# ErickRosete/tacorl

Hardware: AMD Instinct MI355X
Metric: offline grad-steps/sec (batch=256, 84x84 RGB) (higher is better)
Workload: dtype bf16; 1 GPU; tacorl actor-critic training_step, frozen LMP (BASELINE configs[1]); per_gpu_batch=256, global_batch=256, window=16, image=84x84x3, frames=fp32 CHW (reference batch schema), latent_plan=16, n_action_samples=4, phase=Q (epoch>=bc_epochs), action_decoder_loss=every step (reference behaviour), parallelism=dp1, hip_graph=True, losses_finite=True

## Files before the change

include/tacorl_hip.h:

```cpp
#ifndef TACORL_HIP_H
#define TACORL_HIP_H
#include <stddef.h>
#ifdef __cplusplus
extern "C" {
#endif

typedef void* tacorl_stream_t;

#define TACORL_MAXP 16
enum { TACORL_F32 = 0, TACORL_BF16 = 1 };
enum { TACORL_ACT_NONE = 0, TACORL_ACT_RELU = 1, TACORL_ACT_SILU = 2, TACORL_ACT_TANH = 3 };

int tacorl_hip_version(void);
int tacorl_hip_init(int device);
const char* tacorl_hip_last_error(void);
int tacorl_time_mark(unsigned long long* marks, int slot, tacorl_stream_t stream);
int tacorl_time_spin(unsigned long long* marks, int slot, long ticks, tacorl_stream_t stream);

int tacorl_linear_fwd(int nprob, const float* const* x, int ldx, const float* const* w,
                      const float* const* b, float* const* y, float* const* z, const int* M,
                      int K, int N, int act, int compute_dtype, tacorl_stream_t stream);
size_t tacorl_linear_add_fwd_ws_bytes(int nprob, const int* M, int K, int N);
int tacorl_linear_add_fwd(int nprob, const float* const* x, int ldx, const float* const* w,
                          const float* const* b, const float* const* addend, int ld_add, float* const* y,
// ... 105 lines not shown
int tacorl_encoder_bwd_fused_head(int nprob, const float* const* params, const float* const* act,
                                  const float* const* d_out, const int* n_img, int H, int W,
                                  int prepacked, void* ws, size_t ws_bytes, tacorl_stream_t stream);
int tacorl_encoder_bwd_fused_fc_wgrad(int nprob, const float* const* act, const float* const* d_out,
                                      float* const* grads, const int* n_img, int H, int W,
                                      int accumulate, void* ws, size_t ws_bytes, tacorl_stream_t stream);
int tacorl_encoder_bwd_fused_conv(int nprob, const void* const* img, const float* const* params,
                                  const float* const* act, float* const* grads, const int* n_img, int H,
                                  int W, int accumulate, int prepacked, void* ws, size_t ws_bytes,
                                  tacorl_stream_t stream);
int tacorl_encoder_bwd_fused_conv_parts(int nprob, const void* const* img, const float* const* params,
                                        const float* const* act, float* const* grads, const int* n_img, int H,
                                        int W, int accumulate, int prepacked, int parts, void* ws,
                                        size_t ws_bytes, tacorl_stream_t stream);

long tacorl_mlp_param_layout(int n_layers, const int* dims, long* w_off, long* b_off);
long tacorl_mlp_act_layout(int M, int n_layers, const int* dims, const int* acts, long* z_off,
                           long* y_off);
int tacorl_mlp_fwd(int nprob, const float* const* x, int ldx, const float* const* params,
                   float* const* act, const int* M, int n_layers, const int* dims,
                   const int* acts, int compute_dtype, tacorl_stream_t stream);
int tacorl_mlp_fwd_fused_supported(int nprob, int n_layers, const int* dims, int ldx);
int tacorl_mlp_lean_supported(int nprob, int n_layers, const int* dims, int ldx, int ldo, int ldd);
int tacorl_mlp_fwd_fused(int nprob, const float* const* x, int ldx, const float* const* params,
                         const void* const* params_bf16, float* const* act, const int* M,
                         int n_layers, const int* dims, const int* acts, int lean, tacorl_stream_t stream);
int tacorl_mlp_fwd_fused_gather_supported(int nprob, const int* M, int n_layers, const int* dims, const int* acts,
                                          int ldx, int lean);
int tacorl_mlp_fwd_fused_gather(int nprob, const int* nseg, const float* const* seg_ptr, const int* seg_ld,
                                const int* seg_c0, const int* seg_mod, float* const* x_out, int ldx,
                                const float* const* params, const void* const* params_bf16, float* const* act,
                                const int* M, int n_layers, const int* dims, const int* acts, int lean,
                                tacorl_stream_t stream);
int tacorl_to_bf16_batch(int n, const float* const* src, void* const* dst, const long* count,
                         tacorl_stream_t stream);
size_t tacorl_mlp_bwd_ws_bytes(int nprob, const int* M, int n_layers, const int* dims);
int tacorl_mlp_bwd(int nprob, const float* const* x, int ldx, const float* const* params,
                   const float* const* act, const float* const* d_out, int ldo, float* const* grads,
                   float* const* d_x, int ldd, const int* M, int n_layers, const int* dims,
                   const int* acts, int compute_dtype, int accumulate, void* ws, size_t ws_bytes,
                   tacorl_stream_t stream);
int tacorl_mlp_bwd_fused_supported(int nprob, int n_layers, const int* dims, int ldo, int ldd);
size_t tacorl_mlp_bwd_fused_ws_bytes(int nprob, const int* M, int n_layers, const int* dims);
int tacorl_mlp_bwd_fused_dgrad(int nprob, const float* const* params, const float* const* act,
                               const float* const* d_out, int ldo, float* const* d_x, int ldd,
                               const int* M, int n_layers, const int* dims, const int* acts,
                               int prepacked, void* ws, size_t ws_bytes, tacorl_stream_t stream);
int tacorl_mlp_bwd_fused_pack(int nprob, const float* const* params, const int* M, int n_layers,
                              const int* dims, void* ws, size_t ws_bytes, tacorl_stream_t stream);
int tacorl_prep_batch_begin(void);
int tacorl_reduce_batch_begin(void);
int tacorl_reduce_batch_end(tacorl_stream_t stream);
int tacorl_prep_batch_end(tacorl_stream_t stream);
int tacorl_mlp_bwd_fused_wgrad(int nprob, const float* const* x, int ldx, const float* const* act,
                               const float* const* d_out, int ldo, float* const* grads, const int* M,
                               int n_layers, const int* dims, const int* acts, int accumulate, int lean,
                               void* ws, size_t ws_bytes, tacorl_stream_t stream);

int tacorl_pack_images(const float* src, long img_pitch, int src_nchw, void* dst, int dst_dtype,
                       int n, int C, int H, int W, tacorl_stream_t stream);
int tacorl_pack_images_batch(int njobs, const float* const* src, const long* img_pitch, void* const* dst,
                             const int* n_img, int dst_dtype, int H, int W, tacorl_stream_t stream);
int tacorl_pack_images_window_batch(int njobs, const float* const* src, const long* img_pitch, void* const* dst,
                                    const int* n_img, void* const* dst_first, void* const* dst_last,
                                    const int* window, int dst_dtype, int H, int W, tacorl_stream_t stream);
int tacorl_pack_images_u8_batch(int njobs, const void* const* src, const long* img_pitch_bytes, void* const* dst,
                                const int* n_img, int dst_dtype, int H, int W, tacorl_stream_t stream);
int tacorl_pack_images_u8_gather_batch(int njobs, const void* const* src, const long* img_pitch_bytes,
                                       const long* const* index, const int* index_stride, void* const* dst,
                                       const int* n_img, int dst_dtype, int H, int W, tacorl_stream_t stream);
int tacorl_gather_frames_u8(const void* frames, long frame_bytes, const long* index, void* dst, long n,
                            tacorl_stream_t stream);
int tacorl_pack_images_u8_aug_batch(int njobs, const void* const* src, const long* img_pitch_bytes,
                                    void* const* dst, const int* const* shift, const float* const* jitter,
                                    const int* n_img, int dst_dtype, int H, int W, int pad,
                                    tacorl_stream_t stream);
int tacorl_pack_images_u8_resize_aug_gather_batch(int njobs, const void* const* src, const long* img_pitch_bytes,
                                                  const long* const* index, const int* index_stride, void* const* dst,
                                                  const int* const* shift, const float* const* jitter, const int* n_img,
                                                  int dst_dtype, int src_H, int src_W, int H, int W, int pad,
                                                  tacorl_stream_t stream);
int tacorl_pack_images_u8_aug_gather_batch(int njobs, const void* const* src, const long* img_pitch_bytes,
                                           const long* const* index, const int* index_stride, void* const* dst,
                                           const int* const* shift, const float* const* jitter, const int* n_img,
                                           int dst_dtype, int H, int W, int pad, tacorl_stream_t stream);
int tacorl_stage_transition(const void* disp, int disp_dtype, float* reward, float* done, int B,
                            const float* acts_src, float* acts_dst, long n_acts, tacorl_stream_t stream);
int tacorl_sample_transitions(const long* possible_steps, long n_possible, const long* ep_start, const long* ep_end,
                              int n_episodes, const long* nn_ptr, long n_nn, const long* nn_val, const float* actions,
                              const long* idx, const long* strategy, const long* disp, const double* u_choice,
                              long current_horizon, long n_frames, int B, int A, long* ids, float* action,
                              float* reward, float* done, int* status, tacorl_stream_t stream);
int tacorl_sample_relay(const long* episode_lookup, long n_items, const long* ep_start, const long* ep_end, int n_episodes,
                        const float* actions, long n_frames, const long* idx, const double* u_low, const double* u_high,
                        long max_low_level_window, long max_high_level_window, int B, int A, long* ids, float* action,
                        int* status, tacorl_stream_t stream);
int tacorl_sample_d4rl_windows(const long* episode_lookup, long n_items, const long* ep_start, const long* ep_end,
                               int n_episodes, const float* observations, const float* actions, long n_frames,
                               const long* idx, const long* window, const long* disp, int B, int Tmax, int S, int A,
                               int G, int min_window, float threshold, float* obs, float* act, float* goal,
                               float* reached, float* done, long* window_size, long* ids, int* status,
                               tacorl_stream_t stream);
int tacorl_sample_play_windows(const long* episode_lookup, long n_items, const long* ep_start, const long* ep_end,
                               int n_episodes, const long* nn_ptr, long n_nn, const long* nn_val, const float* actions,
                               long n_frames, long last_end, const long* idx, const long* window, const long* strategy,
                               const long* disp, const long* noise_step, const double* u_choice,
                               const double* u_random_state, int B, int Tmax, int A, int min_window, long* ids, float* act,
                               long* disp_out, long* window_size, int* status, tacorl_stream_t stream);
int tacorl_copy_cols(const float* src, int ld_src, float* dst, int ld_dst, int rows, int cols,
                     int src_row_mod, int accumulate, tacorl_stream_t stream);
int tacorl_copy_cols_batch(int n, const float* const* src, const int* ld_src, float* const* dst,
                           const int* ld_dst, const int* rows, const int* cols,
                           const int* src_row_mod, const int* accumulate, tacorl_stream_t stream);
int tacorl_vec_rows_max_blocks(void);
int tacorl_vec_rows(const float* obs, const float* goal, const float* acts_main, const float* act_pi,
                    const float* act_next, float* const* out, void* const* out_bf16, int B, int T, int S, int G, int A,
                    int n, int lds, int ldq, tacorl_stream_t stream);
int tacorl_reduce_rows_mod(const float* in, int ld_in, float* out, int ld_out, int B, int cols,
                           int reps, tacorl_stream_t stream);
int tacorl_reduce_rows_mod_batch(int n, const float* const* in, int ld_in, float* const* out, int ld_out, int B,
                                 int cols, int reps, tacorl_stream_t stream);
int tacorl_uniform_actions(const float* u01, float* dst, int ld_dst, int rows, int A,
                           int discrete_gripper, tacorl_stream_t stream);

int tacorl_tanh_normal_sample(const float* head, int ld_head, const float* eps, const float* gumbel_u,
                              int hard_rsample, float* act_out, int ld_act, float* logp, int* grip_idx,
                              int n, int M, int Ac, tacorl_stream_t stream);
int tacorl_tanh_normal_sample_batch(int njobs, const float* const* head, int ld_head,
                                    const float* const* eps, const float* const* gumbel_u,
                                    const int* hard_rsample, float* const* act_out, int ld_act,
                                    float* const* logp, int* const* grip_idx, const int* n, int M, int Ac,
                                    const float* u01, float* u_dst, int u_rows, int A, int u_discrete,
                                    tacorl_stream_t stream);

int tacorl_add_rows_bcast(const float* x, int ldx, const float* add, float* out, int R, int T, int D,
                          int Dp, tacorl_stream_t stream);
int tacorl_attention_fwd(const float* qkv, float* out, int B, int T, int D, int H, tacorl_stream_t stream);
int tacorl_attention_dropout_fwd(const float* qkv, float* out, const unsigned char* keep, float keep_scale, int B,
                                 int T, int D, int H, tacorl_stream_t stream);
int tacorl_attention_dropout_bwd(const float* qkv, const float* d_out, float* d_qkv, const unsigned char* keep,
                                 float keep_scale, int B, int T, int D, int H, tacorl_stream_t stream);
int tacorl_dropout_mul(float* x, const unsigned char* keep, float keep_scale, long n, tacorl_stream_t stream);
int tacorl_add_layernorm_fwd(const float* x, const float* res, const float* w, const float* b, float* y,
                             float* stats, int R, int D, float eps, tacorl_stream_t stream);
int tacorl_pr_encoder_fused_supported(int D, int T, int H, int FF, int L);
int tacorl_pr_encoder_fused_train_supported(int D, int T, int H, int FF, int L);
int tacorl_pr_encoder_fused(const float* emb, int ld_emb, const float* params, const void* params_bf16,
                            const long* offsets, float* pooled, int B, int D, int T, int H, int FF, int L,
                            tacorl_stream_t stream);
int tacorl_pr_encoder_fused_sample(const float* emb, int ld_emb, const float* params, const void* params_bf16,
                                   const long* offsets, float* pooled, int B, int D, int T, int H, int FF, int L,
                                   const float* Wc, const float* bc, const float* eps, float* head, float* plan,
                                   int A, float min_std, tacorl_stream_t stream);
int tacorl_pr_encoder_fused_train(const float* emb, int ld_emb, const float* params, const void* params_bf16,
                                  const long* offsets, float* pooled, int B, int D, int T, int H, int FF, int L,
                                  float* const* save, tacorl_stream_t stream);
int tacorl_pr_encoder_bwd_fused(const float* params, const long* offsets, const float* d_pool, const float* d_head,
                                const float* Wc, int A2, float* dx, const float* const* saved, float* const* dz,
                                const void* const* wt, float* ln_part, float* const* ln_grads, int B, int D, int T, int H,
                                int FF, int L, tacorl_stream_t stream);
int tacorl_pr_encoder_fused_train_sample(const float* emb, int ld_emb, const float* params, const void* params_bf16,
                                         const long* offsets, float* pooled, int B, int D, int T, int H, int FF, int L,
                                         float* const* save, const float* Wc, const float* bc, const float* eps,
                                         float* head, float* plan, int A, float min_std, tacorl_stream_t stream);
int tacorl_pr_head_compose(const float* w_fc, const float* b_fc, const float* w_head, const float* b_head,
                           float* Wc, float* bc, int D, int FC, int A2, tacorl_stream_t stream);
int tacorl_mean_over_t(const float* x, float* out, int B, int T, int D, tacorl_stream_t stream);
int tacorl_pr_sample(const float* head, const float* eps, float* plan, float* mu_out, float* std_out,
                     int B, int A, float min_std, tacorl_stream_t stream);

int tacorl_build_ad_input(const float* plan, const float* emb, int ld_emb, float* out, int B, int T,
                          int Tm, int P, int E, tacorl_stream_t stream);
int tacorl_ad_input_proj(const float* plan, const float* emb, int ld_emb, const float* w_ih, const float* b_ih,
                         float* out, int B, int T, int Tm, int P, int E, int H, tacorl_stream_t stream);
size_t tacorl_logistic_mixture_ws_bytes(int B, int Tm, int Da);
int tacorl_logistic_mixture_loss(const float* heads, int ldh, const float* actions, float* d_heads,
                                 float* loss_out, int B, int T, int Tm, int Da, int K, int num_classes,
                                 float gripper_alpha, float grad_scale, void* ws, size_t ws_bytes,
                                 tacorl_stream_t stream);
int tacorl_logistic_mixture_finish(const void* ws, size_t ws_bytes, int B, int Tm, int Da, float* loss_out,
                                   tacorl_stream_t stream);
int tacorl_logistic_mixture_sample(const float* heads, int ldh, const float* rand_a, const float* rand_b,
                                   float* out, int R, int Da, int K, tacorl_stream_t stream);

int tacorl_logistic_mixture_nogrip_loss(const float* heads, int ldh, const float* actions, float* d_heads,
                                        float* loss_out, int B, int T, int Tm, int Da, int K, int num_classes,
                                        float grad_scale, void* ws, size_t ws_bytes, tacorl_stream_t stream);
int tacorl_logistic_mixture_nogrip_finish(const void* ws, size_t ws_bytes, int B, int Tm, int Da, float* loss_out,
                                          tacorl_stream_t stream);
int tacorl_logistic_mixture_nogrip_sample(const float* heads, int ldh, const float* rand_a, const float* rand_b,
                                          float* out, int R, int Da, int K, tacorl_stream_t stream);

int tacorl_relu_mask_mul(const float* dy, const float* add, const float* h, float* out, long n,
                         tacorl_stream_t stream);
int tacorl_ad_input_bwd(const float* dx, float* d_plan, float* d_emb, int ld_emb, int B, int T, int Tm,
                        int P, int E, int accumulate, tacorl_stream_t stream);
int tacorl_plmp_demb_finish(float* d_emb, const float* dx, int ld_dx, int D_in, const float* dS, int ld_ds,
                            const float* dgin, float* const* f_dout, int ncam, int B, int T, int Ec,
                            tacorl_stream_t stream);
int tacorl_bcast_over_t(const float* src, float* dst, int B, int T, int D, float scale, int accumulate,
                        tacorl_stream_t stream);
int tacorl_attention_bwd(const float* qkv, const float* d_out, float* d_qkv, int B, int T, int D, int H,
                         tacorl_stream_t stream);
size_t tacorl_add_layernorm_bwd_ws_bytes(int R, int D);
int tacorl_add_layernorm_bwd(const float* dy, const float* x, const float* res, const float* w,
                             const float* stats, float* dv, float* dw, float* db, int R, int D,
                             int accumulate, void* ws, size_t ws_bytes, tacorl_stream_t stream);
int tacorl_gauss_kl_balanced(const float* head_q, const float* head_p, float* d_head_q, float* d_head_p,
                             int B, int A, float kl_alpha, float kl_beta, float min_std, int balanced,
                             float grad_scale, float* out2, tacorl_stream_t stream);
int tacorl_pr_sample_bwd(const float* head, const float* eps, const float* d_plan, float* d_head, int B,
                         int A, float min_std, tacorl_stream_t stream);

enum {
  TACORL_LG_ALPHA_LOSS = 0, TACORL_LG_ALPHA, TACORL_LG_ACTOR_LOSS, TACORL_LG_BELL1, TACORL_LG_BELL2,
  TACORL_LG_CONS1, TACORL_LG_CONS2, TACORL_LG_Q1LOSS, TACORL_LG_Q2LOSS, TACORL_LG_ALPHA_P,
  TACORL_LG_ALPHA_P_LOSS, TACORL_LG_Q1_DATA, TACORL_LG_Q1_RAND, TACORL_LG_Q1_POL, TACORL_LG_Q2_DATA,
  TACORL_LG_Q2_RAND, TACORL_LG_Q2_POL, TACORL_LG_ACTION_LOSS, TACORL_LG_COUNT
};
int tacorl_alpha_loss(const float* logp, int B, const float* log_alpha, float target_entropy,
                      float grad_scale, float* g_log_alpha, float* logs, tacorl_stream_t stream);
int tacorl_alpha_loss_step(const float* logp, int B, float* log_alpha, float target_entropy, float* g_log_alpha,
                           float* logs, float* m, float* v, float lr, int* step_counter, tacorl_stream_t stream);
int tacorl_actor_qmin(const float* q1, const float* q2, const float* logp, int B, const float* log_alpha,
                      float* dq1, float* dq2, float grad_scale, float* logs, tacorl_stream_t stream);
int tacorl_actor_head_bwd(const float* head, int ld_head, const float* eps, const float* logp,
                          const float* g_act1, const float* g_act2, int ld_g, const float* value,
                          int ld_value, const int* grip_idx, const float* log_alpha, float grad_scale,
                          float* d_head, int B, int Ac, int has_grip, float* logs, tacorl_stream_t stream);
int tacorl_tanh_normal_nll(const float* head, int ld_head, const float* target, int ld_target, int M, int Ac,
                           int has_grip, float grad_scale, float* d_head, float* loss_out, tacorl_stream_t stream);

size_t tacorl_cql_ws_bytes(int B);
int tacorl_cql_loss(const float* q1, const float* q2, float* dq1, float* dq2, const float* tq1,
                    const float* tq2, const float* logp_cur, const float* logp_nxt, const float* next_logp,
                    const float* reward, const float* done, const float* log_alpha,
                    const float* log_alpha_prime, int B, int n, int A, float discount, float reward_scale,
                    float temp, float cons_w, float gap, int deterministic_backup, float grad_scale,
                    float* g_log_alpha_prime, float* logs, void* ws, size_t ws_bytes, tacorl_stream_t stream);

size_t tacorl_adam_ws_bytes(long n);
int tacorl_adam_step(float* param, const float* grad, float* m, float* v, long n, float lr,
                     float max_norm, int* step_counter, float* target, float tau, void* ws,
                     size_t ws_bytes, tacorl_stream_t stream);
size_t tacorl_adam_batch_ws_bytes(int nb);
int tacorl_adam_step_batch(int nb, float* const* param, const float* const* grad, float* const* m,
                           float* const* v, const long* n, const float* lr, const float* max_norm,
                           int* const* step_counter, float* const* target, const float* tau, void* ws,
                           size_t ws_bytes, tacorl_stream_t stream);
int tacorl_adam_step_batch_mirror(int nb, float* const* param, const float* const* grad, float* const* m,
                                  float* const* v, const long* n, const float* lr, const float* max_norm,
                                  int* const* step_counter, float* const* target, const float* tau,
                                  void* const* mirror, void* const* target_mirror, void* ws, size_t ws_bytes,
                                  tacorl_stream_t stream);

int tacorl_cem_supported(int N, int A, int E, int hidden, int q_layers, int compute_dtype);
size_t tacorl_cem_ws_bytes(int R, int N, int A, int E, int hidden, int q_layers, int compute_dtype);
int tacorl_cem_refine(int R, int nnet, const float* const* s, const float* const* params,
                      const void* const* params_bf16, const float* mean0, const float* eps, float* out, int N, int A,
                      int E, int hidden, int q_layers, int iters, int n_elite, float min_std, float max_std, float alpha,
                      int discrete_gripper, int compute_dtype, float* t_pop, float* t_q, int* t_elite, float* t_mean,
                      float* t_std, void* ws, size_t ws_bytes, tacorl_stream_t stream);

int tacorl_knn_l2_supported(int D, int k);
int tacorl_knn_l2_tile(void);
int tacorl_knn_l2_query_block(int k);
int tacorl_knn_l2(const float* points, long n_points, int D, long ld, long q0, long n_queries, int k, int* nbr_row,
                  float* nbr_dist, tacorl_stream_t stream);
int tacorl_nn_margin_filter(const int* nbr_row, long n_queries, int k, long q0, const long* step_of_row, long n_points,
                            long margin, long* nn_steps, int* count, tacorl_stream_t stream);

int tacorl_rows_linear2_supported(int R, int K1, int K2, int N);
int tacorl_rows_linear2_group(void);
int tacorl_rows_linear2_fwd(const float* x1, int ldx1, int K1, const float* w1, const float* b1, const float* x2, int ldx2,
                            int K2, const float* w2, const float* b2, const unsigned char* x2_row_is_zero, float* y, int ldy,
                            int R, int N, int act, tacorl_stream_t stream);

#define TACORL_ROWS_MLP_PLAIN 0
#define TACORL_ROWS_MLP_POLICY_ACTION 1
int tacorl_rows_mlp_supported(int R, int n_layers, const int* dims, int mode, int Ac, int discrete_gripper);
int tacorl_rows_mlp_npw(int N, int R);
int tacorl_rows_mlp_fwd(const float* x, int ldx, int n_layers, const int* dims, const float* const* w, const float* const* b,
                        const int* acts, float* ws, float* y, int ldy, int R, int mode, int Ac, int discrete_gripper, int npw,
                        tacorl_stream_t stream);

#define TACORL_NOISE_MAX_SEGS 64
enum { TACORL_NOISE_NORMAL = 0, TACORL_NOISE_UNIFORM = 1, TACORL_NOISE_KEEP = 2 };
typedef struct {
  int offset, kind, draw_id, n_outer, B_local, inner, outer_major;
  float keep_p;
  int group0, reserved;
} tacorl_noise_seg;
typedef struct {
  int n_f32, n_u8, n_groups, reserved;
  tacorl_noise_seg seg[1];
} tacorl_noise_table;
int tacorl_noise_fill(const void* segs, int n_seg, void* base_f32, void* base_u8, unsigned long long seed, unsigned int step,
                      int sample0, tacorl_stream_t stream);

#ifdef __cplusplus
}
#endif
#endif
```

tacorl_amd/_lib.py:

```python
import ctypes as C
import os

HERE = os.path.dirname(os.path.abspath(__file__))
LIB_PATH = os.environ.get("TACORL_HIP_LIB") or os.path.join(HERE, "lib", "libtacorl_hip.so")

F32, BF16 = 0, 1
ACT_NONE, ACT_RELU, ACT_SILU, ACT_TANH = 0, 1, 2, 3
MAXP = 16

LOG_SLOTS = [
    "alpha_loss", "alpha", "actor_loss", "bellman_q1_loss", "bellman_q2_loss", "conservative_q1_loss",
    "conservative_q2_loss", "q1_loss", "q2_loss", "alpha_prime", "alpha_prime_loss", "q1_data", "q1_random",
    "q1_policy", "q2_data", "q2_random", "q2_policy", "action_loss",
]

_p, _i, _l, _f, _sz = C.c_void_p, C.c_int, C.c_long, C.c_float, C.c_size_t
_SIGS = {
    "tacorl_hip_version": (_i, []),
    "tacorl_hip_init": (_i, [_i]),
    "tacorl_hip_last_error": (C.c_char_p, []),
    "tacorl_time_mark": (_i, [_p, _i, _p]),
    "tacorl_time_spin": (_i, [_p, _i, _l, _p]),
    "tacorl_linear_fwd": (_i, [_i, _p, _i, _p, _p, _p, _p, _p, _i, _i, _i, _i, _p]),
    "tacorl_linear_add_fwd_ws_bytes": (_sz, [_i, _p, _i, _i]),
    "tacorl_linear_add_fwd": (_i, [_i, _p, _i, _p, _p, _p, _i, _p, _i, _p, _i, _i, _i, _i, _p, _sz, _p]),
    "tacorl_rnn_linear_supported": (_i, [_i, _i, _i]),
    "tacorl_rnn_linear_fwd": (_i, [_p, _p, _p, _p, _i, _p, _p, _i, _i, _i, _i, _p]),
    "tacorl_rnn_linear_fwd_batch": (_i, [_i, _p, _p, _p, _p, _i, _p, _p, _i, _i, _i, _p, _p]),
    "tacorl_rnn_linear_fwd_batch_twin": (_i, [_i, _p, _p, _p, _p, _p, _p, _i, _p, _p, _p, _p, _i, _i, _i, _i, _p, _p]),
    "tacorl_rnn_linear_fwd_batch_ext": (_i, [_i, _p, _p, _p, _p, _p, _p, _i, _p, _p, _p, _p, _i, _i, _i, _i, _p, _p, _p, _p, _p, _p]),
    "tacorl_rnn_linear_ld_supported": (_i, [_i, _i, _i, _i, _i]),
    "tacorl_rnn_linear_ld": (_i, [_i, _p, _i, _p, _p, _p, _p, _i, _p, _p, _p, _p, _p, _i, _i, _i, _i, _i, _p]),
    "tacorl_rnn_linear_bwd_step": (_i, [_p, _p, _p, _i, _p, _p, _p, _i, _i, _i, _p]),
    "tacorl_rnn_linear_bwd_batch": (_i, [_i, _p, _p, _p, _i, _p, _p, _p, _i, _i, _i, _p]),
    "tacorl_rnn_wgrad_supported": (_i, [_i, _i, _i]),
    "tacorl_rnn_wgrad": (_i, [_p, _i, _p, _i, _i, _i, _i, _p, _p, _i, _p]),
    "tacorl_rnn_wgrad_batch": (_i, [_i, _p, _i, _p, _i, _p, _i, _i, _p, _p, _i, _p]),
    "tacorl_rnn_wgrad_slabs_ws_bytes": (_sz, [_i, _i, _i]),
    "tacorl_rnn_wgrad_slabs": (_i, [_p, _i, _p, _i, _i, _i, _i, _i, _i, _p, _p, _i, _p, _sz, _p]),
    "tacorl_birnn_swap_rows": (_i, [_p, _i, _p, _i, _i, _i, _i, _p]),
    "tacorl_transpose_to_bf16": (_i, [_p, _p, _i, _i, _p]),
    "tacorl_transpose_to_bf16_batch": (_i, [_i, _p, _p, _p, _p, _p]),
    "tacorl_transpose_pad_to_bf16": (_i, [_p, _p, _i, _i, _i, _p]),
    "tacorl_pad_to_bf16": (_i, [_p, _i, _p, _i, _l, _i, _p]),
    "tacorl_pr_encoder_fused_supported": (_i, [_i, _i, _i, _i, _i]),
    "tacorl_pr_encoder_fused_train_supported": (_i, [_i, _i, _i, _i, _i]),
    "tacorl_pr_encoder_fused": (_i, [_p, _i, _p, _p, _p, _p, _i, _i, _i, _i, _i, _i, _p]),
    "tacorl_pr_encoder_fused_train": (_i, [_p, _i, _p, _p, _p, _p, _i, _i, _i, _i, _i, _i, _p, _p]),
    "tacorl_pr_encoder_bwd_fused": (_i, [_p, _p, _p, _p, _p, _i, _p, _p, _p, _p, _p, _p, _i, _i, _i, _i, _i, _i, _p]),
    "tacorl_pr_encoder_fused_train_sample": (_i, [_p, _i, _p, _p, _p, _p, _i, _i, _i, _i, _i, _i, _p, _p, _p, _p, _p, _p, _i, _f, _p]),
    "tacorl_pr_encoder_fused_sample": (_i, [_p, _i, _p, _p, _p, _p, _i, _i, _i, _i, _i, _i, _p, _p, _p, _p, _p, _i, _f, _p]),
    "tacorl_pr_head_compose": (_i, [_p, _p, _p, _p, _p, _p, _i, _i, _i, _p]),
    "tacorl_to_bf16_batch": (_i, [_i, _p, _p, _p, _p]),
    "tacorl_mlp_bwd_fused_supported": (_i, [_i, _i, _p, _i, _i]),
    "tacorl_mlp_bwd_fused_ws_bytes": (_sz, [_i, _p, _i, _p]),
    "tacorl_mlp_bwd_fused_dgrad": (_i, [_i, _p, _p, _p, _i, _p, _i, _p, _i, _p, _p, _i, _p, _sz, _p]),
    "tacorl_mlp_bwd_fused_pack": (_i, [_i, _p, _p, _i, _p, _p, _sz, _p]),
    "tacorl_prep_batch_begin": (_i, []),
    "tacorl_reduce_batch_begin": (_i, []),
    "tacorl_reduce_batch_end": (_i, [_p]),
    "tacorl_prep_batch_end": (_i, [_p]),
    "tacorl_mlp_bwd_fused_wgrad": (_i, [_i, _p, _i, _p, _p, _i, _p, _p, _i, _p, _p, _i, _i, _p, _sz, _p]),
    "tacorl_mlp_fwd_fused_supported": (_i, [_i, _i, _p, _i]),
    "tacorl_mlp_lean_supported": (_i, [_i, _i, _p, _i, _i, _i]),
    "tacorl_mlp_fwd_fused": (_i, [_i, _p, _i, _p, _p, _p, _p, _i, _p, _p, _i, _p]),
    "tacorl_mlp_fwd_fused_gather_supported": (_i, [_i, _p, _i, _p, _p, _i, _i]),
    "tacorl_mlp_fwd_fused_gather": (_i, [_i, _p, _p, _p, _p, _p, _p, _i, _p, _p, _p, _p, _i, _p, _p, _i, _p]),
    "tacorl_add_rows_bcast": (_i, [_p, _i, _p, _p, _i, _i, _i, _i, _p]),
    "tacorl_attention_fwd": (_i, [_p, _p, _i, _i, _i, _i, _p]),
    "tacorl_attention_dropout_fwd": (_i, [_p, _p, _p, _f, _i, _i, _i, _i, _p]),
    "tacorl_attention_dropout_bwd": (_i, [_p, _p, _p, _p, _f, _i, _i, _i, _i, _p]),
    "tacorl_dropout_mul": (_i, [_p, _p, _f, _l, _p]),
    "tacorl_add_layernorm_fwd": (_i, [_p, _p, _p, _p, _p, _p, _i, _i, _f, _p]),
    "tacorl_mean_over_t": (_i, [_p, _p, _i, _i, _i, _p]),
    "tacorl_pr_sample": (_i, [_p, _p, _p, _p, _p, _i, _i, _f, _p]),
    "tacorl_build_ad_input": (_i, [_p, _p, _i, _p, _i, _i, _i, _i, _i, _p]),
    "tacorl_build_ad_input_bf16": (_i, [_p, _p, _i, _p, _i, _i, _i, _i, _i, _p]),
    "tacorl_ad_input_proj": (_i, [_p, _p, _i, _p, _p, _p, _i, _i, _i, _i, _i, _i, _p]),
    "tacorl_logistic_mixture_ws_bytes": (_sz, [_i, _i, _i]),
    "tacorl_logistic_mixture_loss": (_i, [_p, _i, _p, _p, _p, _i, _i, _i, _i, _i, _i, _f, _f, _p, _sz, _p]),
    "tacorl_logistic_mixture_finish": (_i, [_p, _sz, _i, _i, _i, _p, _p]),
    "tacorl_logistic_mixture_sample": (_i, [_p, _i, _p, _p, _p, _i, _i, _i, _p]),
    "tacorl_logistic_mixture_nogrip_loss": (_i, [_p, _i, _p, _p, _p, _i, _i, _i, _i, _i, _i, _f, _p, _sz, _p]),
    "tacorl_logistic_mixture_nogrip_finish": (_i, [_p, _sz, _i, _i, _i, _p, _p]),
    "tacorl_logistic_mixture_nogrip_sample": (_i, [_p, _i, _p, _p, _p, _i, _i, _i, _p]),
    "tacorl_linear_dgrad": (_i, [_i, _p, _i, _p, _p, _i, _p, _i, _i, _p, _i, _p, _i, _i, _i, _p]),
    "tacorl_linear_dgrad_ws_bytes": (_sz, [_i, _p, _i, _i]),
    "tacorl_linear_dgrad_splitk": (_i, [_i, _p, _i, _p, _p, _i, _p, _i, _i, _p, _i, _p, _i, _i, _i, _p, _sz, _p]),
    "tacorl_linear_wgrad_ws_bytes": (_sz, [_i, _p, _i, _i]),
    "tacorl_linear_wgrad": (_i, [_i, _p, _i, _p, _i, _p, _i, _i, _p, _p, _i, _i, _p, _sz, _p]),
    "tacorl_relu_mask_mul": (_i, [_p, _p, _p, _p, _l, _p]),
    "tacorl_ad_input_bwd": (_i, [_p, _p, _p, _i, _i, _i, _i, _i, _i, _i, _p]),
    "tacorl_plmp_demb_finish": (_i, [_p, _p, _i, _i, _p, _i, _p, _p, _i, _i, _i, _i, _p]),
    "tacorl_bcast_over_t": (_i, [_p, _p, _i, _i, _i, _f, _i, _p]),
    "tacorl_attention_bwd": (_i, [_p, _p, _p, _i, _i, _i, _i, _p]),
    "tacorl_add_layernorm_bwd_ws_bytes": (_sz, [_i, _i]),
    "tacorl_add_layernorm_bwd": (_i, [_p, _p, _p, _p, _p, _p, _p, _p, _i, _i, _i, _p, _sz, _p]),
    "tacorl_gauss_kl_balanced": (_i, [_p, _p, _p, _p, _i, _i, _f, _f, _f, _i, _f, _p, _p]),
    "tacorl_pr_sample_bwd": (_i, [_p, _p, _p, _p, _i, _i, _f, _p]),
    "tacorl_conv2d_relu_fwd": (_i, [_i, _p, _p, _p, _p, _p, _i, _i, _i, _i, _i, _i, _i, _i, _i, _p]),
    "tacorl_encoder_param_layout": (_l, [_p]),
    "tacorl_encoder_act_layout": (_l, [_i, _i, _i, _p]),
    "tacorl_encoder_fwd": (_i, [_i, _p, _p, _p, _p, _p, _i, _i, _i, _i, _p]),
    "tacorl_encoder_bwd_ws_bytes": (_sz, [_i, _p, _i, _i]),
    "tacorl_encoder_bwd": (_i, [_i, _p, _p, _p, _p, _p, _p, _i, _i, _i, _i, _i, _p, _sz, _p]),
    "tacorl_encoder_fused_wpk_bytes": (_l, []),
    "tacorl_encoder_fused_supported": (_i, [_i, _i]),
    "tacorl_encoder_fused_act_format": (_i, [_i, _i]),
    "tacorl_encoder_pack_weights": (_i, [_i, _p, _p, _p]),
    "tacorl_encoder_fwd_fused": (_i, [_i, _p, _p, _p, _p, _p, _p, _i, _i, _p]),
    "tacorl_encoder_fwd_fused_wg": (_i, [_i, _p, _p, _p, _p, _p, _p, _i, _i, _i, _p]),
    "tacorl_encoder_src_entry_bytes": (_l, []),
    "tacorl_encoder_src_supported": (_i, [_p, _l, _l, _l, _i, _i]),
    "tacorl_encoder_src_fill": (_i, [_p, _i, _p, _p, _p, _p, _i, _i, _p]),
    "tacorl_encoder_fwd_fused_src": (_i, [_i, _p, _p, _p, _p, _p, _p, _p, _i, _i, _i, _p]),
    "tacorl_encoder_bwd_fused_ws_bytes": (_sz, [_i, _p, _i, _i]),
    "tacorl_encoder_bwd_fused": (_i, [_i, _p, _p, _p, _p, _p, _p, _i, _i, _i, _p, _sz, _p]),
    "tacorl_encoder_bwd_fused_pack": (_i, [_i, _p, _p, _i, _i, _p, _sz, _p]),
    "tacorl_encoder_bwd_fused_head": (_i, [_i, _p, _p, _p, _p, _i, _i, _i, _p, _sz, _p]),
    "tacorl_encoder_bwd_fused_fc_wgrad": (_i, [_i, _p, _p, _p, _p, _i, _i, _i, _p, _sz, _p]),
    "tacorl_encoder_bwd_fused_conv": (_i, [_i, _p, _p, _p, _p, _p, _i, _i, _i, _i, _p, _sz, _p]),
    "tacorl_encoder_bwd_fused_conv_parts": (_i, [_i, _p, _p, _p, _p, _p, _i, _i, _i, _i, _i, _p, _sz, _p]),
    "tacorl_mlp_param_layout": (_l, [_i, _p, _p, _p]),
    "tacorl_mlp_act_layout": (_l, [_i, _i, _p, _p, _p, _p]),
    "tacorl_mlp_fwd": (_i, [_i, _p, _i, _p, _p, _p, _i, _p, _p, _i, _p]),
    "tacorl_mlp_bwd_ws_bytes": (_sz, [_i, _p, _i, _p]),
    "tacorl_mlp_bwd": (_i, [_i, _p, _i, _p, _p, _p, _i, _p, _p, _i, _p, _i, _p, _p, _i, _i, _p, _sz, _p]),
    "tacorl_pack_images": (_i, [_p, _l, _i, _p, _i, _i, _i, _i, _i, _p]),
    "tacorl_pack_images_batch": (_i, [_i, _p, _p, _p, _p, _i, _i, _i, _p]),
    "tacorl_pack_images_window_batch": (_i, [_i, _p, _p, _p, _p, _p, _p, _p, _i, _i, _i, _p]),
    "tacorl_pack_images_u8_batch": (_i, [_i, _p, _p, _p, _p, _i, _i, _i, _p]),
    "tacorl_pack_images_u8_gather_batch": (_i, [_i, _p, _p, _p, _p, _p, _p, _i, _i, _i, _p]),
    "tacorl_pack_images_u8_aug_gather_batch": (_i, [_i, _p, _p, _p, _p, _p, _p, _p, _p, _i, _i, _i, _i, _p]),
    "tacorl_pack_images_u8_resize_aug_gather_batch": (_i, [_i, _p, _p, _p, _p, _p, _p, _p, _p, _i, _i, _i, _i, _i, _i, _p]),
    "tacorl_gather_frames_u8": (_i, [_p, _l, _p, _p, _l, _p]),
    "tacorl_pack_images_u8_aug_batch": (_i, [_i, _p, _p, _p, _p, _p, _p, _i, _i, _i, _i, _p]),
    "tacorl_stage_transition": (_i, [_p, _i, _p, _p, _i, _p, _p, _l, _p]),
    "tacorl_sample_transitions": (_i, [_p, _l, _p, _p, _i, _p, _l, _p, _p, _p, _p, _p, _p, _l, _l, _i, _i, _p, _p, _p, _p, _p, _p]),
    "tacorl_sample_relay": (_i, [_p, _l, _p, _p, _i, _p, _l, _p, _p, _p, _l, _l, _i, _i, _p, _p, _p, _p]),
    "tacorl_sample_d4rl_windows": (_i, [_p, _l, _p, _p, _i, _p, _p, _l, _p, _p, _p, _i, _i, _i, _i, _i, _i, _f, _p, _p, _p, _p, _p, _p,
                                        _p, _p, _p]),
    "tacorl_sample_play_windows": (_i, [_p, _l, _p, _p, _i, _p, _l, _p, _p, _l, _l, _p, _p, _p, _p, _p, _p, _p, _i, _i, _i, _i,
                                        _p, _p, _p, _p, _p, _p]),
    "tacorl_copy_cols": (_i, [_p, _i, _p, _i, _i, _i, _i, _i, _p]),
    "tacorl_copy_cols_batch": (_i, [_i, _p, _p, _p, _p, _p, _p, _p, _p, _p]),
    "tacorl_vec_rows_max_blocks": (_i, []),
    "tacorl_vec_rows": (_i, [_p, _p, _p, _p, _p, _p, _p, _i, _i, _i, _i, _i, _i, _i, _i, _p]),
    "tacorl_reduce_rows_mod": (_i, [_p, _i, _p, _i, _i, _i, _i, _p]),
    "tacorl_reduce_rows_mod_batch": (_i, [_i, _p, _i, _p, _i, _i, _i, _i, _p]),
    "tacorl_uniform_actions": (_i, [_p, _p, _i, _i, _i, _i, _p]),
    "tacorl_tanh_normal_sample": (_i, [_p, _i, _p, _p, _i, _p, _i, _p, _p, _i, _i, _i, _p]),
    "tacorl_tanh_normal_sample_batch": (_i, [_i, _p, _i, _p, _p, _p, _p, _i, _p, _p, _p, _i, _i, _p, _p, _i, _i, _i, _p]),
    "tacorl_alpha_loss": (_i, [_p, _i, _p, _f, _f, _p, _p, _p]),
    "tacorl_alpha_loss_step": (_i, [_p, _i, _p, _f, _p, _p, _p, _p, _f, _p, _p]),
    "tacorl_actor_qmin": (_i, [_p, _p, _p, _i, _p, _p, _p, _f, _p, _p]),
    "tacorl_actor_head_bwd": (_i, [_p, _i, _p, _p, _p, _p, _i, _p, _i, _p, _p, _f, _p, _i, _i, _i, _p, _p]),
    "tacorl_tanh_normal_nll": (_i, [_p, _i, _p, _i, _i, _i, _i, _f, _p, _p, _p]),
    "tacorl_cql_ws_bytes": (_sz, [_i]),
    "tacorl_cql_loss": (_i, [_p] * 13 + [_i, _i, _i, _f, _f, _f, _f, _f, _i, _f, _p, _p, _p, _sz, _p]),
    "tacorl_adam_ws_bytes": (_sz, [_l]),
    "tacorl_adam_step": (_i, [_p, _p, _p, _p, _l, _f, _f, _p, _p, _f, _p, _sz, _p]),
    "tacorl_adam_batch_ws_bytes": (_sz, [_i]),
    "tacorl_adam_step_batch": (_i, [_i, _p, _p, _p, _p, _p, _p, _p, _p, _p, _p, _p, _sz, _p]),
    "tacorl_adam_step_batch_mirror": (_i, [_i, _p, _p, _p, _p, _p, _p, _p, _p, _p, _p, _p, _p, _p, _sz, _p]),
    "tacorl_cem_supported": (_i, [_i, _i, _i, _i, _i, _i]),
    "tacorl_cem_ws_bytes": (_sz, [_i, _i, _i, _i, _i, _i, _i]),
    "tacorl_cem_refine": (_i, [_i, _i, _p, _p, _p, _p, _p, _p, _i, _i, _i, _i, _i, _i, _i, _f, _f, _f, _i, _i, _p, _p, _p, _p, _p,
                               _p, _sz, _p]),
    "tacorl_knn_l2_supported": (_i, [_i, _i]),
    "tacorl_knn_l2_tile": (_i, []),
    "tacorl_knn_l2_query_block": (_i, [_i]),
    "tacorl_knn_l2": (_i, [_p, _l, _i, _l, _l, _l, _i, _p, _p, _p]),
    "tacorl_nn_margin_filter": (_i, [_p, _l, _i, _l, _p, _l, _l, _p, _p, _p]),
    "tacorl_rows_linear2_supported": (_i, [_i, _i, _i, _i]),
    "tacorl_rows_linear2_group": (_i, []),
    "tacorl_rows_linear2_fwd": (_i, [_p, _i, _i, _p, _p, _p, _i, _i, _p, _p, _p, _p, _i, _i, _i, _i, _p]),
    "tacorl_rows_mlp_supported": (_i, [_i, _i, _p, _i, _i, _i]),
    "tacorl_rows_mlp_npw": (_i, [_i, _i]),
    "tacorl_rows_mlp_fwd": (_i, [_p, _i, _i, _p, _p, _p, _p, _p, _p, _i, _i, _i, _i, _i, _i, _p]),
    "tacorl_noise_fill": (_i, [_p, _i, _p, _p, C.c_ulonglong, C.c_uint, _i, _p]),
}

_lib = None


class TacorlHipError(RuntimeError):
    pass


def lib():
    global _lib
    if _lib is None:
        import torch

        if not os.path.exists(LIB_PATH):
            raise TacorlHipError(
                f"{LIB_PATH} not found: the HIP extension is required (no CPU fallback). "
                "Build it with `python -m tacorl_amd.build`.")
        L = C.CDLL(LIB_PATH)
        override = bool(os.environ.get("TACORL_HIP_LIB"))
        missing = []
        for name, (res, args) in _SIGS.items():
            fn = getattr(L, name, None)
            if fn is None:
# ... 53 lines not shown
```

tacorl_amd/csrc/pr_fused.hip:

```cpp
#include <hip/hip_runtime.h>
#include <stdint.h>

#include "../../include/tacorl_hip.h"
#include "common.h"

namespace {

#ifndef PR_W2TOP
#define PR_W2TOP 0
#endif
constexpr int PR_D = 32, PR_T = 16, PR_H = 8, PR_HD = 4, PR_MAXL = 4, PR_CH = 256;
constexpr int XB_P = 40;
constexpr int HB_P = 264;
constexpr int QKV_P = 100;

struct PrLayerOff { long in_w, in_b, out_w, out_b, w1, b1, w2, b2, n1w, n1b, n2w, n2b; };
struct PrSaveL { float *xin, *qkv, *att, *proj, *x1, *ff1, *ff2, *st1, *st2; };
struct PrArgs {
  const float* emb;
  const float* P;
  const __bf16* Pb;
  float* pooled;
  long pos;
  PrLayerOff l[PR_MAXL];
  int ld_emb, B, FF, L;
  const float* Wc;
  const float* bc;
  const float* eps;
  float* head;
  float* plan;
  int A;
  float min_std;
  PrSaveL sv[PR_MAXL];
  int save;
};

__device__ __forceinline__ bf16x8 cvt8(const float* p) {
  const f32x4 a = *reinterpret_cast<const f32x4*>(p), b = *reinterpret_cast<const f32x4*>(p + 4);
  return bf16x8{(__bf16)a[0], (__bf16)a[1], (__bf16)a[2], (__bf16)a[3], (__bf16)b[0], (__bf16)b[1], (__bf16)b[2], (__bf16)b[3]};
}
__device__ __forceinline__ void lds_sync() { asm volatile("s_waitcnt lgkmcnt(0)" ::: "memory"); }

__device__ __forceinline__ void layer_norm32(f32x4 (&v)[2], const float* w, const float* b, int g, float* st = nullptr) {
  float s = 0.f;
#pragma unroll
  for (int nt = 0; nt < 2; nt++)
#pragma unroll
    for (int r = 0; r < 4; r++) s += v[nt][r];
  s += __shfl_xor(s, 16, 64);
  s += __shfl_xor(s, 32, 64);
  const float mean = s / 32.f;
  float q = 0.f;
#pragma unroll
  for (int nt = 0; nt < 2; nt++)
#pragma unroll
    for (int r = 0; r < 4; r++) { const float c = v[nt][r] - mean; q += c * c; }
  q += __shfl_xor(q, 16, 64);
  q += __shfl_xor(q, 32, 64);
  const float rstd = 1.0f / sqrtf(q / 32.f + 1e-5f);
  if (st && g == 0) { st[0] = mean; st[1] = rstd; }
#pragma unroll
  for (int nt = 0; nt < 2; nt++) {
    const f32x4 ww = *reinterpret_cast<const f32x4*>(w + 16 * nt + 4 * g), bb = *reinterpret_cast<const f32x4*>(b + 16 * nt + 4 * g);
#pragma unroll
    for (int r = 0; r < 4; r++) v[nt][r] = (v[nt][r] - mean) * rstd * ww[r] + bb[r];
  }
}

__device__ __forceinline__ void layer_norm32_r(f32x4 (&v)[2], const f32x4 (&ww)[2], const f32x4 (&bb)[2], int g, float* st = nullptr) {
  float s = 0.f;
#pragma unroll
  for (int nt = 0; nt < 2; nt++)
#pragma unroll
    for (int r = 0; r < 4; r++) s += v[nt][r];
  s += __shfl_xor(s, 16, 64);
  s += __shfl_xor(s, 32, 64);
  const float mean = s / 32.f;
  float q = 0.f;
#pragma unroll
  for (int nt = 0; nt < 2; nt++)
#pragma unroll
    for (int r = 0; r < 4; r++) { const float c = v[nt][r] - mean; q += c * c; }
  q += __shfl_xor(q, 16, 64);
  q += __shfl_xor(q, 32, 64);
  const float rstd = 1.0f / sqrtf(q / 32.f + 1e-5f);
  if (st && g == 0) { st[0] = mean; st[1] = rstd; }
#pragma unroll
  for (int nt = 0; nt < 2; nt++)
#pragma unroll
    for (int r = 0; r < 4; r++) v[nt][r] = (v[nt][r] - mean) * rstd * ww[nt][r] + bb[nt][r];
}

#ifdef PR_STAMPS
__device__ unsigned long long pr_stamps[16];
#define PR_STAMP(k)                                          \
  do {                                                       \
    if (blockIdx.x == 0 && threadIdx.x == 0) {               \
      const unsigned long long t_ = clock64();               \
      atomicAdd(&pr_stamps[k], t_ - t_prev);                 \
      t_prev = t_;                                           \
    }                                                        \
  } while (0)
#else
#define PR_STAMP(k)
#endif

template <int RT>
__global__ __launch_bounds__(256) void pr_encoder_fused_kernel(PrArgs a) {
#ifdef PR_STAMPS
  unsigned long long t_prev = clock64();
#endif
  constexpr int T = 16 * RT;
  __shared__ __attribute__((aligned(16))) __bf16 xb_s[4][T * XB_P];
  __shared__ __attribute__((aligned(16))) unsigned char big_s[4][T * HB_P * 2];
  const int lane = threadIdx.x & 63, w = threadIdx.x >> 6, i = lane & 15, g = lane >> 4;
  __shared__ __attribute__((aligned(16))) float ypart[2][4][T * PR_D];
  constexpr int PR_B1C = 2;
  __shared__ __attribute__((aligned(16))) float b1_s[4][PR_B1C * PR_CH];
  const int b = blockIdx.x;
  if (b >= a.B) return;
  __bf16* xb = xb_s[w];
  float* qkv = reinterpret_cast<float*>(big_s[w]);
  __bf16* hb = reinterpret_cast<__bf16*>(big_s[w]);
  static_assert(T * QKV_P * 4 <= T * HB_P * 2, "q|k|v fits in the hidden-chunk buffer");

  const int A_ = a.A, jh = lane < 2 * A_ ? lane : 0;
  f32x4 hw[PR_D / 4];
  float hbias = 0.f, heps = 0.f;
  if (a.Wc) {
#pragma unroll
    for (int d = 0; d < PR_D / 4; d++) hw[d] = *reinterpret_cast<const f32x4*>(a.Wc + jh * PR_D + 4 * d);
    hbias = a.bc[jh];
    heps = a.eps[(long)b * A_ + (lane < A_ ? lane : 0)];
  }
  f32x4 x[RT][2];
#pragma unroll
  for (int rt = 0; rt < RT; rt++)
#pragma unroll
    for (int nt = 0; nt < 2; nt++) {
      const int n = 16 * nt + 4 * g, t = 16 * rt + i;
      x[rt][nt] = *reinterpret_cast<const f32x4*>(a.emb + ((long)b * T + t) * a.ld_emb + n) +
                  *reinterpret_cast<const f32x4*>(a.P + a.pos + t * PR_D + n);
    }
  auto put_xb = [&](const f32x4 (&v)[RT][2]) {
#pragma unroll
    for (int rt = 0; rt < RT; rt++)
#pragma unroll
      for (int nt = 0; nt < 2; nt++)
        *reinterpret_cast<bf16x4*>(xb + (16 * rt + i) * XB_P + 16 * nt + 4 * g) =
            bf16x4{(__bf16)v[rt][nt][0], (__bf16)v[rt][nt][1], (__bf16)v[rt][nt][2], (__bf16)v[rt][nt][3]};
  };
  const int nchunk = a.FF / PR_CH;
  const bool sv0 = a.save && w == 0;
  long rrow[RT];
#pragma unroll
  for (int rt = 0; rt < RT; rt++) rrow[rt] = (long)b * T + 16 * rt + i;
  for (int l = 0; l < a.L; l++) {
    const PrLayerOff& o = a.l[l];
    const PrSaveL& S = a.sv[l];
    bf16x8 inw[6], outw[2];
    f32x4 inb[6], outb[2], n1w[2], n1b[2], n2w[2], n2b[2], b2v[2];
#pragma unroll
    for (int nt = 0; nt < 6; nt++) {
      inw[nt] = *reinterpret_cast<const bf16x8*>(a.Pb + o.in_w + (long)(16 * nt + i) * PR_D + 8 * g);
      inb[nt] = *reinterpret_cast<const f32x4*>(a.P + o.in_b + 16 * nt + 4 * g);
    }
#pragma unroll
    for (int nt = 0; nt < 2; nt++) {
      outw[nt] = *reinterpret_cast<const bf16x8*>(a.Pb + o.out_w + (long)(16 * nt + i) * PR_D + 8 * g);
      outb[nt] = *reinterpret_cast<const f32x4*>(a.P + o.out_b + 16 * nt + 4 * g);
      n1w[nt] = *reinterpret_cast<const f32x4*>(a.P + o.n1w + 16 * nt + 4 * g);
      n1b[nt] = *reinterpret_cast<const f32x4*>(a.P + o.n1b + 16 * nt + 4 * g);
      n2w[nt] = *reinterpret_cast<const f32x4*>(a.P + o.n2w + 16 * nt + 4 * g);
      n2b[nt] = *reinterpret_cast<const f32x4*>(a.P + o.n2b + 16 * nt + 4 * g);
      b2v[nt] = *reinterpret_cast<const f32x4*>(a.P + o.b2 + 16 * nt + 4 * g);
    }
    const __bf16* W1 = a.Pb + o.w1;
    const __bf16* W2 = a.Pb + o.w2;
    bf16x8 w1f[16], w2f[8][2];
    const int c0 = w < nchunk ? w : nchunk - 1;
#pragma unroll
    for (int nt = 0; nt < 16; nt++) w1f[nt] = *reinterpret_cast<const bf16x8*>(W1 + (long)(PR_CH * c0 + 16 * nt + i) * PR_D + 8 * g);
    f32x4 b1pre[PR_B1C];
    const bool b1_staged = nchunk <= 4 * PR_B1C;
    if (b1_staged) {
#pragma unroll
      for (int j = 0; j < PR_B1C; j++) {
        const int c = w + 4 * j;
        b1pre[j] = *reinterpret_cast<const f32x4*>(a.P + o.b1 + PR_CH * (c < nchunk ? c : c0) + 4 * lane);
      }
    }
    if (RT == 1 && PR_W2TOP) {
#pragma unroll
      for (int ks = 0; ks < 8; ks++)
#pragma unroll
        for (int nt = 0; nt < 2; nt++)
          w2f[ks][nt] = *reinterpret_cast<const bf16x8*>(W2 + (long)(16 * nt + i) * a.FF + PR_CH * c0 + 32 * ks + 8 * g);
    }
    if (sv0) {
#pragma unroll
      for (int rt = 0; rt < RT; rt++)
#pragma unroll
        for (int nt = 0; nt < 2; nt++) *reinterpret_cast<f32x4*>(S.xin + rrow[rt] * PR_D + 16 * nt + 4 * g) = x[rt][nt];
    }
    PR_STAMP(0);
    put_xb(x);
    lds_sync();
    {
      bf16x8 xf[RT];
#pragma unroll
      for (int rt = 0; rt < RT; rt++) xf[rt] = *reinterpret_cast<const bf16x8*>(xb + (16 * rt + i) * XB_P + 8 * g);
#pragma unroll
      for (int nt = 0; nt < 6; nt++) {
        const bf16x8 wf = inw[nt];
        const f32x4 bias = inb[nt];
#pragma unroll
        for (int rt = 0; rt < RT; rt++) {
          f32x4 acc = bias;
          acc = __builtin_amdgcn_mfma_f32_16x16x32_bf16(wf, xf[rt], acc, 0, 0, 0);
          *reinterpret_cast<f32x4*>(qkv + (16 * rt + i) * QKV_P + 16 * nt + 4 * g) = acc;
          if (sv0) *reinterpret_cast<f32x4*>(S.qkv + rrow[rt] * 3 * PR_D + 16 * nt + 4 * g) = acc;
        }
      }
    }
    lds_sync();
    PR_STAMP(1);
#pragma unroll
    for (int j = 0; j < 2 * RT; j++) {
      const int p = lane + 64 * j, h = p / T, qi = p % T;
      f32x4 q = *reinterpret_cast<const f32x4*>(qkv + qi * QKV_P + PR_HD * h);
#pragma unroll
      for (int e = 0; e < 4; e++) q[e] *= 0.5f * 1.44269504088896341f;
      float s[T], mx = -INFINITY;
#pragma unroll
      for (int t = 0; t < T; t++) {
        const f32x4 k = *reinterpret_cast<const f32x4*>(qkv + t * QKV_P + PR_D + PR_HD * h);
        s[t] = ((q[0] * k[0] + q[1] * k[1]) + q[2] * k[2]) + q[3] * k[3];
        mx = fmaxf(mx, s[t]);
      }
      float se = 0.f;
#pragma unroll
      for (int t = 0; t < T; t++) { s[t] = __builtin_amdgcn_exp2f(s[t] - mx); se += s[t]; }
      const float rse = __builtin_amdgcn_rcpf(se);
      f32x4 ov = {0.f, 0.f, 0.f, 0.f};
#pragma unroll
      for (int t = 0; t < T; t++) {
        const f32x4 vv = *reinterpret_cast<const f32x4*>(qkv + t * QKV_P + 2 * PR_D + PR_HD * h);
        const float pr = s[t] * rse;
#pragma unroll
        for (int e = 0; e < 4; e++) ov[e] += pr * vv[e];
      }
      *reinterpret_cast<bf16x4*>(xb + qi * XB_P + PR_HD * h) = bf16x4{(__bf16)ov[0], (__bf16)ov[1], (__bf16)ov[2], (__bf16)ov[3]};
      if (sv0) *reinterpret_cast<f32x4*>(S.att + ((long)b * T + qi) * PR_D + PR_HD * h) = ov;
    }
    lds_sync();
    PR_STAMP(2);
    {
      bf16x8 af[RT];
#pragma unroll
      for (int rt = 0; rt < RT; rt++) af[rt] = *reinterpret_cast<const bf16x8*>(xb + (16 * rt + i) * XB_P + 8 * g);
#pragma unroll
      for (int nt = 0; nt < 2; nt++) {
        const bf16x8 wf = outw[nt];
        const f32x4 bias = outb[nt];
#pragma unroll
        for (int rt = 0; rt < RT; rt++) {
          f32x4 acc = bias;
          acc = __builtin_amdgcn_mfma_f32_16x16x32_bf16(wf, af[rt], acc, 0, 0, 0);
          if (sv0) *reinterpret_cast<f32x4*>(S.proj + rrow[rt] * PR_D + 16 * nt + 4 * g) = acc;
          x[rt][nt] += acc;
        }
      }
#pragma unroll
      for (int rt = 0; rt < RT; rt++) {
        layer_norm32_r(x[rt], n1w, n1b, g, sv0 ? S.st1 + 2 * rrow[rt] : nullptr);
        if (sv0) {
#pragma unroll
          for (int nt = 0; nt < 2; nt++) *reinterpret_cast<f32x4*>(S.x1 + rrow[rt] * PR_D + 16 * nt + 4 * g) = x[rt][nt];
        }
      }
    }
    lds_sync();
    put_xb(x);
    lds_sync();
    PR_STAMP(3);
    if (b1_staged) {
#pragma unroll
      for (int j = 0; j < PR_B1C; j++) *reinterpret_cast<f32x4*>(b1_s[w] + PR_CH * j + 4 * lane) = b1pre[j];
      lds_sync();
    }
    bf16x8 xf[RT];
#pragma unroll
    for (int rt = 0; rt < RT; rt++) xf[rt] = *reinterpret_cast<const bf16x8*>(xb + (16 * rt + i) * XB_P + 8 * g);
    f32x4 y[RT][2];
#pragma unroll
    for (int rt = 0; rt < RT; rt++)
#pragma unroll
      for (int nt = 0; nt < 2; nt++)
        y[rt][nt] = w == 0 ? b2v[nt] : f32x4{0.f, 0.f, 0.f, 0.f};
    for (int c = w; c < nchunk; c += 4) {
      if (RT != 1 || !PR_W2TOP || c != w) {
#pragma unroll
        for (int ks = 0; ks < 8; ks++)
#pragma unroll
          for (int nt = 0; nt < 2; nt++)
            w2f[ks][nt] = *reinterpret_cast<const bf16x8*>(W2 + (long)(16 * nt + i) * a.FF + PR_CH * c + 32 * ks + 8 * g);
      }
#pragma unroll
      for (int nt = 0; nt < 16; nt++) {
        const f32x4 bias = b1_staged ? *reinterpret_cast<const f32x4*>(b1_s[w] + PR_CH * ((c - w) >> 2) + 16 * nt + 4 * g)
                                     : *reinterpret_cast<const f32x4*>(a.P + o.b1 + PR_CH * c + 16 * nt + 4 * g);
#pragma unroll
        for (int rt = 0; rt < RT; rt++) {
          f32x4 hacc = bias;
          hacc = __builtin_amdgcn_mfma_f32_16x16x32_bf16(w1f[nt], xf[rt], hacc, 0, 0, 0);
          const f32x4 hr = {fmaxf(hacc[0], 0.f), fmaxf(hacc[1], 0.f), fmaxf(hacc[2], 0.f), fmaxf(hacc[3], 0.f)};
          *reinterpret_cast<bf16x4*>(hb + (16 * rt + i) * HB_P + 16 * nt + 4 * g) = bf16x4{(__bf16)hr[0], (__bf16)hr[1], (__bf16)hr[2], (__bf16)hr[3]};
          if (a.save) *reinterpret_cast<f32x4*>(S.ff1 + rrow[rt] * a.FF + PR_CH * c + 16 * nt + 4 * g) = hr;
        }
      }
      lds_sync();
      if (c + 4 < nchunk) {
#pragma unroll
        for (int nt = 0; nt < 16; nt++)
          w1f[nt] = *reinterpret_cast<const bf16x8*>(W1 + (long)(PR_CH * (c + 4) + 16 * nt + i) * PR_D + 8 * g);
      }
#pragma unroll
      for (int ks = 0; ks < 8; ks++) {
#pragma unroll
        for (int rt = 0; rt < RT; rt++) {
          const bf16x8 hf = *reinterpret_cast<const bf16x8*>(hb + (16 * rt + i) * HB_P + 32 * ks + 8 * g);
#pragma unroll
          for (int nt = 0; nt < 2; nt++) y[rt][nt] = __builtin_amdgcn_mfma_f32_16x16x32_bf16(w2f[ks][nt], hf, y[rt][nt], 0, 0, 0);
        }
      }
      lds_sync();
    }
    PR_STAMP(4);
    {
      float* yp = ypart[l & 1][w];
#pragma unroll
      for (int rt = 0; rt < RT; rt++)
#pragma unroll
        for (int nt = 0; nt < 2; nt++) *reinterpret_cast<f32x4*>(yp + (16 * rt + i) * PR_D + 16 * nt + 4 * g) = y[rt][nt];
      __syncthreads();
#pragma unroll
      for (int rt = 0; rt < RT; rt++)
#pragma unroll
        for (int nt = 0; nt < 2; nt++) {
          f32x4 t = *reinterpret_cast<const f32x4*>(ypart[l & 1][0] + (16 * rt + i) * PR_D + 16 * nt + 4 * g);
#pragma unroll
          for (int ww = 1; ww < 4; ww++) t += *reinterpret_cast<const f32x4*>(ypart[l & 1][ww] + (16 * rt + i) * PR_D + 16 * nt + 4 * g);
          if (sv0) *reinterpret_cast<f32x4*>(S.ff2 + rrow[rt] * PR_D + 16 * nt + 4 * g) = t;
          x[rt][nt] += t;
        }
    }
#pragma unroll
    for (int rt = 0; rt < RT; rt++) layer_norm32_r(x[rt], n2w, n2b, g, sv0 ? S.st2 + 2 * rrow[rt] : nullptr);
    PR_STAMP(5);
  }
  if (w != 0) return;
#pragma unroll
  for (int nt = 0; nt < 2; nt++) {
    f32x4 s = x[0][nt];
#pragma unroll
    for (int rt = 1; rt < RT; rt++) s += x[rt][nt];
#pragma unroll
    for (int off = 1; off < 16; off <<= 1)
#pragma unroll
      for (int r = 0; r < 4; r++) s[r] += __shfl_xor(s[r], off, 64);
    if (i == 0) {
#pragma unroll
      for (int r = 0; r < 4; r++) s[r] *= (1.0f / T);
      *reinterpret_cast<f32x4*>(a.pooled + (long)b * PR_D + 16 * nt + 4 * g) = s;
      if (a.Wc) *reinterpret_cast<f32x4*>(qkv + 16 * nt + 4 * g) = s;
    }
  }
  if (!a.Wc) return;
  lds_sync();
  const int A = A_;
  float h = hbias;
#pragma unroll
  for (int d = 0; d < PR_D; d += 4) {
    const f32x4 wv = hw[d / 4], pv = *reinterpret_cast<const f32x4*>(qkv + d);
    h += wv[0] * pv[0] + wv[1] * pv[1] + wv[2] * pv[2] + wv[3] * pv[3];
  }
  if (lane < 2 * A) a.head[(long)b * 2 * A + lane] = h;
  const float vr = __shfl(h, (lane + A) & 63, 64);
  if (lane < A) {
    const float sd = (vr > 20.f ? vr : log1pf(expf(vr))) + a.min_std;
    a.plan[(long)b * A + lane] = tanhf(h + heps * sd);
  }
}

constexpr int D6 = 64, HD6 = 8, CH6 = 128;
constexpr int XB6_P = 72;
constexpr int HB6_P = 136;
constexpr int QKV6_P = 196;

__device__ __forceinline__ void layer_norm64(f32x4 (&v)[4], const float* w, const float* b, int g) {
  float s = 0.f;
#pragma unroll
  for (int nt = 0; nt < 4; nt++)
#pragma unroll
    for (int r = 0; r < 4; r++) s += v[nt][r];
  s += __shfl_xor(s, 16, 64);
  s += __shfl_xor(s, 32, 64);
  const float mean = s / 64.f;
  float q = 0.f;
#pragma unroll
  for (int nt = 0; nt < 4; nt++)
#pragma unroll
    for (int r = 0; r < 4; r++) { const float c = v[nt][r] - mean; q += c * c; }
  q += __shfl_xor(q, 16, 64);
  q += __shfl_xor(q, 32, 64);
  const float rstd = 1.0f / sqrtf(q / 64.f + 1e-5f);
#pragma unroll
  for (int nt = 0; nt < 4; nt++) {
    const f32x4 ww = *reinterpret_cast<const f32x4*>(w + 16 * nt + 4 * g), bb = *reinterpret_cast<const f32x4*>(b + 16 * nt + 4 * g);
#pragma unroll
    for (int r = 0; r < 4; r++) v[nt][r] = (v[nt][r] - mean) * rstd * ww[r] + bb[r];
  }
}

__device__ __forceinline__ void layer_norm64(f32x4 (&v)[4], const f32x4 (&ww)[4], const f32x4 (&bb)[4]) {
  float s = 0.f;
#pragma unroll
  for (int nt = 0; nt < 4; nt++)
#pragma unroll
    for (int r = 0; r < 4; r++) s += v[nt][r];
  s += __shfl_xor(s, 16, 64);
  s += __shfl_xor(s, 32, 64);
  const float mean = s / 64.f;
  float q = 0.f;
#pragma unroll
  for (int nt = 0; nt < 4; nt++)
#pragma unroll
    for (int r = 0; r < 4; r++) { const float c = v[nt][r] - mean; q += c * c; }
  q += __shfl_xor(q, 16, 64);
  q += __shfl_xor(q, 32, 64);
  const float rstd = 1.0f / sqrtf(q / 64.f + 1e-5f);
#pragma unroll
  for (int nt = 0; nt < 4; nt++)
#pragma unroll
    for (int r = 0; r < 4; r++) v[nt][r] = (v[nt][r] - mean) * rstd * ww[nt][r] + bb[nt][r];
}

template <int RT>
__global__ __launch_bounds__(256) void pr_encoder_fused64_kernel(PrArgs a) {
#ifdef PR_STAMPS
  unsigned long long t_prev = clock64();
#endif
  constexpr int T = 16 * RT;
  constexpr int BIG = (T * QKV6_P * 4 > T * HB6_P * 2) ? T * QKV6_P * 4 : T * HB6_P * 2;
  __shared__ __attribute__((aligned(16))) __bf16 xb_s[4][T * XB6_P];
  __shared__ __attribute__((aligned(16))) unsigned char big_s[4][BIG];
  __shared__ __attribute__((aligned(16))) float ypart[4][T * D6];
  __shared__ __attribute__((aligned(16))) __bf16 xatt[T * XB6_P];
  const int lane = threadIdx.x & 63, w = threadIdx.x >> 6, i = lane & 15, g = lane >> 4;
  const int b = blockIdx.x;
  if (b >= a.B) return;
  __bf16* xb = xb_s[w];
  float* qkv = reinterpret_cast<float*>(big_s[w]);
  __bf16* hb = reinterpret_cast<__bf16*>(big_s[w]);
  f32x4 x[RT][4];
#pragma unroll
  for (int rt = 0; rt < RT; rt++)
#pragma unroll
    for (int nt = 0; nt < 4; nt++) {
      const int n = 16 * nt + 4 * g, t = 16 * rt + i;
      x[rt][nt] = *reinterpret_cast<const f32x4*>(a.emb + ((long)b * T + t) * a.ld_emb + n) +
                  *reinterpret_cast<const f32x4*>(a.P + a.pos + t * D6 + n);
    }
  auto put_xb = [&](const f32x4 (&v)[RT][4]) {
#pragma unroll
    for (int rt = 0; rt < RT; rt++)
#pragma unroll
      for (int nt = 0; nt < 4; nt++)
        *reinterpret_cast<bf16x4*>(xb + (16 * rt + i) * XB6_P + 16 * nt + 4 * g) =
            bf16x4{(__bf16)v[rt][nt][0], (__bf16)v[rt][nt][1], (__bf16)v[rt][nt][2], (__bf16)v[rt][nt][3]};
  };
  auto get_xf = [&](bf16x8 (&xf)[RT][2]) {
#pragma unroll
    for (int rt = 0; rt < RT; rt++)
#pragma unroll
      for (int ks = 0; ks < 2; ks++) xf[rt][ks] = *reinterpret_cast<const bf16x8*>(xb + (16 * rt + i) * XB6_P + 32 * ks + 8 * g);
  };
  const int nchunk = a.FF / CH6;
  for (int l = 0; l < a.L; l++) {
    const PrLayerOff& o = a.l[l];
    PR_STAMP(0);
    bf16x8 inw[3][2];
    f32x4 inb[3];
#pragma unroll
    for (int k3 = 0; k3 < 3; k3++) {
      const int nt = 4 * k3 + w;
      inw[k3][0] = *reinterpret_cast<const bf16x8*>(a.Pb + o.in_w + (long)(16 * nt + i) * D6 + 8 * g);
      inw[k3][1] = *reinterpret_cast<const bf16x8*>(a.Pb + o.in_w + (long)(16 * nt + i) * D6 + 32 + 8 * g);
      inb[k3] = *reinterpret_cast<const f32x4*>(a.P + o.in_b + 16 * nt + 4 * g);
    }
    put_xb(x);
    lds_sync();
    {
      bf16x8 xf[RT][2];
      get_xf(xf);
#pragma unroll
      for (int k3 = 0; k3 < 3; k3++) {
        const int nt = 4 * k3 + w;
#pragma unroll
        for (int rt = 0; rt < RT; rt++) {
          f32x4 acc = inb[k3];
          acc = __builtin_amdgcn_mfma_f32_16x16x32_bf16(inw[k3][0], xf[rt][0], acc, 0, 0, 0);
          acc = __builtin_amdgcn_mfma_f32_16x16x32_bf16(inw[k3][1], xf[rt][1], acc, 0, 0, 0);
          *reinterpret_cast<f32x4*>(qkv + (16 * rt + i) * QKV6_P + 16 * nt + 4 * g) = acc;
        }
      }
    }
    bf16x8 outw[4][2];
    f32x4 outb[4], n1w[4], n1b[4];
#pragma unroll
    for (int nt = 0; nt < 4; nt++) {
      outw[nt][0] = *reinterpret_cast<const bf16x8*>(a.Pb + o.out_w + (long)(16 * nt + i) * D6 + 8 * g);
      outw[nt][1] = *reinterpret_cast<const bf16x8*>(a.Pb + o.out_w + (long)(16 * nt + i) * D6 + 32 + 8 * g);
      outb[nt] = *reinterpret_cast<const f32x4*>(a.P + o.out_b + 16 * nt + 4 * g);
      n1w[nt] = *reinterpret_cast<const f32x4*>(a.P + o.n1w + 16 * nt + 4 * g);
      n1b[nt] = *reinterpret_cast<const f32x4*>(a.P + o.n1b + 16 * nt + 4 * g);
    }
    lds_sync();
    PR_STAMP(1);
    {
      const int p = lane & (2 * T - 1), h = 2 * w + p / T, qi = p % T;
      f32x4 q0 = *reinterpret_cast<const f32x4*>(qkv + qi * QKV6_P + HD6 * h), q1 = *reinterpret_cast<const f32x4*>(qkv + qi * QKV6_P + HD6 * h + 4);
      const float sc = 0.35355339059327379f * 1.44269504088896341f;
      q0 *= sc; q1 *= sc;
      float s[T], mx = -INFINITY;
#pragma unroll
      for (int t = 0; t < T; t++) {
        const f32x4 k0 = *reinterpret_cast<const f32x4*>(qkv + t * QKV6_P + D6 + HD6 * h), k1 = *reinterpret_cast<const f32x4*>(qkv + t * QKV6_P + D6 + HD6 * h + 4);
        s[t] = (((q0[0] * k0[0] + q0[1] * k0[1]) + q0[2] * k0[2]) + q0[3] * k0[3]) + (((q1[0] * k1[0] + q1[1] * k1[1]) + q1[2] * k1[2]) + q1[3] * k1[3]);
        mx = fmaxf(mx, s[t]);
      }
      float se = 0.f;
#pragma unroll
      for (int t = 0; t < T; t++) { s[t] = __builtin_amdgcn_exp2f(s[t] - mx); se += s[t]; }
// ... 314 lines not shown
      for (int nt = 0; nt < 2; nt++) *reinterpret_cast<f32x4*>(S.dv1b + rrow * PR_D + 16 * nt + 4 * g) = dv1[nt];
    }
    put_xb(dv1);
    lds_sync();
    {
      const bf16x8 af = *reinterpret_cast<const bf16x8*>(xb + i * XB_P + 8 * g);
#pragma unroll
      for (int nt = 0; nt < 2; nt++) {
        bf16x8 wf;
        if (S.wot) {
          wf = *reinterpret_cast<const bf16x8*>(S.wot + (16 * nt + i) * PR_D + 8 * g);
        } else {
#pragma unroll
          for (int q = 0; q < 8; q++) wf[q] = (__bf16)a.P[o.out_w + (long)(8 * g + q) * PR_D + 16 * nt + i];
        }
        f32x4 acc = {0.f, 0.f, 0.f, 0.f};
        acc = __builtin_amdgcn_mfma_f32_16x16x32_bf16(wf, af, acc, 0, 0, 0);
        *reinterpret_cast<f32x4*>(datt + i * 36 + 16 * nt + 4 * g) = acc;
      }
    }
#pragma unroll
    for (int k = 0; k < 6; k++) {
      const int e = lane + 64 * k, row = e / 24, c4 = e - row * 24;
      *reinterpret_cast<f32x4*>(qkv + row * QKV_P + 4 * c4) = *reinterpret_cast<const f32x4*>(S.qkv + ((long)b * PR_T + row) * 3 * PR_D + 4 * c4);
    }
    lds_sync();
#pragma unroll
    for (int j = 0; j < 2; j++) {
      const int hl = lane >> 4, h = 4 * j + hl, qi = lane & 15;
      float* pp = pm_s[w][hl][0];
      float* pd = pm_s[w][hl][1];
      f32x4 qs = *reinterpret_cast<const f32x4*>(qkv + qi * QKV_P + PR_HD * h);
      qs *= 0.5f;
      const f32x4 dO = *reinterpret_cast<const f32x4*>(datt + qi * 36 + PR_HD * h);
      float ws_[PR_T], dp[PR_T], mx = -INFINITY;
#pragma unroll
      for (int t = 0; t < PR_T; t++) {
        const f32x4 kt = *reinterpret_cast<const f32x4*>(qkv + t * QKV_P + PR_D + PR_HD * h);
        const f32x4 vt = *reinterpret_cast<const f32x4*>(qkv + t * QKV_P + 2 * PR_D + PR_HD * h);
        ws_[t] = ((qs[0] * kt[0] + qs[1] * kt[1]) + qs[2] * kt[2]) + qs[3] * kt[3];
        dp[t] = ((dO[0] * vt[0] + dO[1] * vt[1]) + dO[2] * vt[2]) + dO[3] * vt[3];
        mx = fmaxf(mx, ws_[t]);
      }
      float se = 0.f, dd = 0.f;
#pragma unroll
      for (int t = 0; t < PR_T; t++) { ws_[t] = expf(ws_[t] - mx); se += ws_[t]; dd += ws_[t] * dp[t]; }
      dd /= se;
      f32x4 dq = {0.f, 0.f, 0.f, 0.f};
#pragma unroll
      for (int t = 0; t < PR_T; t++) {
        const float pj = ws_[t] / se, ds = pj * (dp[t] - dd);
        const f32x4 kt = *reinterpret_cast<const f32x4*>(qkv + t * QKV_P + PR_D + PR_HD * h);
        dq += ds * kt;
        pp[qi * 17 + t] = pj;
        pd[qi * 17 + t] = ds;
      }
      lds_sync();
      f32x4 dk = {0.f, 0.f, 0.f, 0.f}, dvv = {0.f, 0.f, 0.f, 0.f};
#pragma unroll
      for (int r = 0; r < PR_T; r++) {
        f32x4 qr = *reinterpret_cast<const f32x4*>(qkv + r * QKV_P + PR_HD * h);
        const f32x4 dor = *reinterpret_cast<const f32x4*>(datt + r * 36 + PR_HD * h);
        qr *= 0.5f;
        dk += pd[r * 17 + qi] * qr;
        dvv += pp[r * 17 + qi] * dor;
      }
      dq *= 0.5f;
      if (sv0) {
        float* dst = S.d_qkv + ((long)b * PR_T + qi) * 3 * PR_D + PR_HD * h;
        *reinterpret_cast<f32x4*>(dst) = dq;
        *reinterpret_cast<f32x4*>(dst + PR_D) = dk;
        *reinterpret_cast<f32x4*>(dst + 2 * PR_D) = dvv;
      }
      __bf16* db_ = dqb + qi * DQ_P + PR_HD * h;
      *reinterpret_cast<bf16x4*>(db_) = bf16x4{(__bf16)dq[0], (__bf16)dq[1], (__bf16)dq[2], (__bf16)dq[3]};
      *reinterpret_cast<bf16x4*>(db_ + PR_D) = bf16x4{(__bf16)dk[0], (__bf16)dk[1], (__bf16)dk[2], (__bf16)dk[3]};
      *reinterpret_cast<bf16x4*>(db_ + 2 * PR_D) = bf16x4{(__bf16)dvv[0], (__bf16)dvv[1], (__bf16)dvv[2], (__bf16)dvv[3]};
      lds_sync();
    }
#pragma unroll
    for (int nt = 0; nt < 2; nt++) {
      f32x4 acc = dv1[nt];
#pragma unroll
      for (int ks = 0; ks < 3; ks++) {
        const bf16x8 df = *reinterpret_cast<const bf16x8*>(dqb + i * DQ_P + 32 * ks + 8 * g);
        bf16x8 wf;
        if (S.wint) {
          wf = *reinterpret_cast<const bf16x8*>(S.wint + (16 * nt + i) * (3 * PR_D) + 32 * ks + 8 * g);
        } else {
#pragma unroll
          for (int q = 0; q < 8; q++) wf[q] = (__bf16)a.P[o.in_w + (long)(32 * ks + 8 * g + q) * PR_D + 16 * nt + i];
        }
        acc = __builtin_amdgcn_mfma_f32_16x16x32_bf16(wf, df, acc, 0, 0, 0);
      }
      dx[nt] = acc;
    }
    lds_sync();
  }
  if (sv0) {
#pragma unroll
    for (int nt = 0; nt < 2; nt++) *reinterpret_cast<f32x4*>(a.dx + rrow * PR_D + 16 * nt + 4 * g) = dx[nt];
  }
}

struct PrLnReduceArgs { const float* part; float* dw[2 * PR_MAXL]; float* db[2 * PR_MAXL]; int B; };
__global__ __launch_bounds__(256) void pr_ln_reduce_kernel(PrLnReduceArgs a) {
  __shared__ float red[4][64];
  const int c = threadIdx.x & 63, ph = threadIdx.x >> 6;
  const float* in = a.part + (long)blockIdx.x * a.B * 64;
  float s = 0.f;
  for (int r = ph; r < a.B; r += 4) s += in[(long)r * 64 + c];
  red[ph][c] = s;
  __syncthreads();
  if (ph == 0) {
    const float t = ((red[0][c] + red[1][c]) + red[2][c]) + red[3][c];
    if (c < 32) a.dw[blockIdx.x][c] = t; else a.db[blockIdx.x][c - 32] = t;
  }
}

__global__ __launch_bounds__(256) void pr_head_compose_kernel(const float* __restrict__ w_fc, const float* __restrict__ b_fc,
                                                              const float* __restrict__ w_head, const float* __restrict__ b_head,
                                                              float* __restrict__ Wc, float* __restrict__ bc, int FC, int D) {
  __shared__ float part[8][64 + 1];
  const int NG = 256 / D;
  const int j = blockIdx.x, d = threadIdx.x % D, fg = threadIdx.x / D;
  float acc = 0.f, accb = 0.f;
#pragma unroll 16
  for (int f = fg; f < FC; f += NG) {
    const float wh = w_head[(long)j * FC + f];
    acc += wh * w_fc[(long)f * D + d];
    accb += wh * b_fc[f];
  }
  part[fg][d] = acc;
  if (d == 0) part[fg][D] = accb;
  __syncthreads();
  if (threadIdx.x <= D) {
    float t = 0.f;
    for (int q = 0; q < NG; q++) t += part[q][threadIdx.x];
    if (threadIdx.x < D) Wc[j * D + threadIdx.x] = t;
    else bc[j] = t + b_head[j];
  }
}

}

extern "C" int tacorl_pr_encoder_fused_supported(int D, int T, int H, int FF, int L) {
  return (D == PR_D || D == D6) && (T == PR_T || T == 2 * PR_T) && H == PR_H && FF >= PR_CH && FF % PR_CH == 0 && L >= 1 &&
                 L <= PR_MAXL
             ? 1 : 0;
}
extern "C" int tacorl_pr_encoder_fused_train_supported(int D, int T, int H, int FF, int L) {
  return D == PR_D && tacorl_pr_encoder_fused_supported(D, T, H, FF, L) ? 1 : 0;
}
static int pr_encoder_fused_launch(const float* emb, int ld_emb, const float* params, const void* params_bf16,
                                   const long* offsets, float* pooled, int B, int D, int T, int H, int FF, int L,
                                   const float* Wc, const float* bc, const float* eps, float* head, float* plan, int A,
                                   float min_std, tacorl_stream_t stream, float* const* save = nullptr) {
  if (!tacorl_pr_encoder_fused_supported(D, T, H, FF, L) || ld_emb % 4 || B < 1) return TACORL_EINVAL;
  if (((uintptr_t)emb | (uintptr_t)params | (uintptr_t)params_bf16 | (uintptr_t)pooled) & 15) return TACORL_EINVAL;
  PrArgs a{};
  a.emb = emb; a.P = params; a.Pb = (const __bf16*)params_bf16; a.pooled = pooled; a.ld_emb = ld_emb; a.B = B; a.FF = FF; a.L = L;
  if (offsets[0] % 4) return TACORL_EINVAL;
  a.pos = offsets[0];
  for (int l = 0; l < L; l++) {
    const long* q = offsets + 1 + 12 * l;
    for (int k = 0; k < 12; k++)
      if (q[k] % 4) return TACORL_EINVAL;
    a.l[l] = PrLayerOff{q[0], q[1], q[2], q[3], q[4], q[5], q[6], q[7], q[8], q[9], q[10], q[11]};
  }
  if (Wc) {
    if (!bc || !eps || !head || !plan || A < 1 || 2 * A > 64 || ((uintptr_t)Wc & 15)) return TACORL_EINVAL;
    a.Wc = Wc; a.bc = bc; a.eps = eps; a.head = head; a.plan = plan; a.A = A; a.min_std = min_std;
  }
  if (save) {
    for (int l = 0; l < L; l++) {
      float* const* q = save + 9 * l;
      for (int k = 0; k < 9; k++)
        if (!q[k] || ((uintptr_t)q[k] & 15)) return TACORL_EINVAL;
      a.sv[l] = PrSaveL{q[0], q[1], q[2], q[3], q[4], q[5], q[6], q[7], q[8]};
    }
    a.save = 1;
  }
  if (D == D6) {
    if (save) return TACORL_EINVAL;
    if (T == PR_T) hipLaunchKernelGGL(pr_encoder_fused64_kernel<1>, dim3(B), dim3(256), 0, (hipStream_t)stream, a);
    else hipLaunchKernelGGL(pr_encoder_fused64_kernel<2>, dim3(B), dim3(256), 0, (hipStream_t)stream, a);
  } else if (T == PR_T) hipLaunchKernelGGL(pr_encoder_fused_kernel<1>, dim3(B), dim3(256), 0, (hipStream_t)stream, a);
  else hipLaunchKernelGGL(pr_encoder_fused_kernel<2>, dim3(B), dim3(256), 0, (hipStream_t)stream, a);
  return hipGetLastError() == hipSuccess ? TACORL_OK : TACORL_ELAUNCH;
}
extern "C" int tacorl_pr_encoder_fused_train(const float* emb, int ld_emb, const float* params, const void* params_bf16,
                                             const long* offsets, float* pooled, int B, int D, int T, int H, int FF, int L,
                                             float* const* save, tacorl_stream_t stream) {
  if (!save) return TACORL_EINVAL;
  return pr_encoder_fused_launch(emb, ld_emb, params, params_bf16, offsets, pooled, B, D, T, H, FF, L, nullptr, nullptr,
                                 nullptr, nullptr, nullptr, 0, 0.f, stream, save);
}
extern "C" int tacorl_pr_encoder_fused_train_sample(const float* emb, int ld_emb, const float* params, const void* params_bf16,
                                                    const long* offsets, float* pooled, int B, int D, int T, int H, int FF,
                                                    int L, float* const* save, const float* Wc, const float* bc,
                                                    const float* eps, float* head, float* plan, int A, float min_std,
                                                    tacorl_stream_t stream) {
  if (!save || !Wc) return TACORL_EINVAL;
  return pr_encoder_fused_launch(emb, ld_emb, params, params_bf16, offsets, pooled, B, D, T, H, FF, L, Wc, bc, eps, head, plan,
                                 A, min_std, stream, save);
}
extern "C" int tacorl_pr_encoder_fused(const float* emb, int ld_emb, const float* params, const void* params_bf16,
                                       const long* offsets, float* pooled, int B, int D, int T, int H, int FF, int L,
                                       tacorl_stream_t stream) {
  return pr_encoder_fused_launch(emb, ld_emb, params, params_bf16, offsets, pooled, B, D, T, H, FF, L, nullptr, nullptr,
                                 nullptr, nullptr, nullptr, 0, 0.f, stream);
}
extern "C" int tacorl_pr_encoder_fused_sample(const float* emb, int ld_emb, const float* params, const void* params_bf16,
                                              const long* offsets, float* pooled, int B, int D, int T, int H, int FF,
                                              int L, const float* Wc, const float* bc, const float* eps, float* head,
                                              float* plan, int A, float min_std, tacorl_stream_t stream) {
  if (!Wc) return TACORL_EINVAL;
  return pr_encoder_fused_launch(emb, ld_emb, params, params_bf16, offsets, pooled, B, D, T, H, FF, L, Wc, bc, eps, head,
                                 plan, A, min_std, stream);
}
extern "C" int tacorl_pr_head_compose(const float* w_fc, const float* b_fc, const float* w_head, const float* b_head,
                                      float* Wc, float* bc, int D, int FC, int A2, tacorl_stream_t stream) {
  if ((D != PR_D && D != D6) || FC < 1 || A2 < 1 || !w_fc || !b_fc || !w_head || !b_head || !Wc || !bc) return TACORL_EINVAL;
  hipLaunchKernelGGL(pr_head_compose_kernel, dim3(A2), dim3(256), 0, (hipStream_t)stream, w_fc, b_fc, w_head, b_head, Wc, bc,
                     FC, D);
  return hipGetLastError() == hipSuccess ? TACORL_OK : TACORL_ELAUNCH;
}

extern "C" int tacorl_pr_encoder_bwd_fused(const float* params, const long* offsets, const float* d_pool, const float* d_head,
                                           const float* Wc, int A2, float* dx, const float* const* saved, float* const* dz,
                                           const void* const* wt, float* ln_part, float* const* ln_grads, int B, int D, int T,
                                           int H, int FF, int L, tacorl_stream_t stream) {
  if (!tacorl_pr_encoder_fused_train_supported(D, T, H, FF, L) || D != PR_D || T != PR_T || B < 1) return TACORL_EINVAL;
  if (!params || !dx || !saved || !dz || !wt || !ln_part || !ln_grads) return TACORL_EINVAL;
  if (!d_pool && (!d_head || !Wc || A2 < 1)) return TACORL_EINVAL;
  if (((uintptr_t)params | (uintptr_t)d_pool | (uintptr_t)dx | (uintptr_t)ln_part | (uintptr_t)Wc) & 15) return TACORL_EINVAL;
  PrBwdArgs a{};
  PrLnReduceArgs r{};
  a.P = params; a.d_pool = d_pool; a.d_head = d_head; a.Wc = Wc; a.A2 = A2; a.dx = dx; a.lnpart = ln_part; a.B = B; a.FF = FF; a.L = L;
  r.part = ln_part; r.B = B;
  for (int l = 0; l < L; l++) {
    const long* q = offsets + 1 + 12 * l;
    for (int k = 0; k < 12; k++)
      if (q[k] % 4) return TACORL_EINVAL;
    a.l[l] = PrLayerOff{q[0], q[1], q[2], q[3], q[4], q[5], q[6], q[7], q[8], q[9], q[10], q[11]};
    const float* const* sv = saved + 9 * l;
    float* const* z = dz + 4 * l;
    for (int k = 0; k < 9; k++)
      if (!sv[k] || ((uintptr_t)sv[k] & 15)) return TACORL_EINVAL;
    for (int k = 0; k < 4; k++)
      if (!z[k] || ((uintptr_t)z[k] & 15) || !ln_grads[4 * l + k]) return TACORL_EINVAL;
    if (!wt[4 * l] || !wt[4 * l + 1] ||
        (((uintptr_t)wt[4 * l] | (uintptr_t)wt[4 * l + 1] | (uintptr_t)wt[4 * l + 2] | (uintptr_t)wt[4 * l + 3]) & 15))
      return TACORL_EINVAL;
    a.s[l] = PrBwdL{sv[0], sv[1], sv[2], sv[3], sv[4], sv[5], sv[6], sv[7], sv[8], z[0], z[1], z[2], z[3],
                    (const __bf16*)wt[4 * l], (const __bf16*)wt[4 * l + 1], (const __bf16*)wt[4 * l + 2], (const __bf16*)wt[4 * l + 3]};
    r.dw[2 * l] = ln_grads[4 * l]; r.db[2 * l] = ln_grads[4 * l + 1];
    r.dw[2 * l + 1] = ln_grads[4 * l + 2]; r.db[2 * l + 1] = ln_grads[4 * l + 3];
  }
  hipLaunchKernelGGL(pr_encoder_bwd_fused_kernel, dim3(B), dim3(256), 0, (hipStream_t)stream, a);
  hipLaunchKernelGGL(pr_ln_reduce_kernel, dim3(2 * L), dim3(256), 0, (hipStream_t)stream, r);
  return hipGetLastError() == hipSuccess ? TACORL_OK : TACORL_ELAUNCH;
}

#ifdef PR_STAMPS
extern "C" int tacorl_pr_stamps_read(unsigned long long* out, int reset) {
  if (hipMemcpyFromSymbol(out, HIP_SYMBOL(pr_stamps), sizeof(pr_stamps)) != hipSuccess) return TACORL_ELAUNCH;
  if (reset) {
    unsigned long long z[16] = {};
    if (hipMemcpyToSymbol(HIP_SYMBOL(pr_stamps), z, sizeof(z)) != hipSuccess) return TACORL_ELAUNCH;
  }
  return TACORL_OK;
}
#endif
```

tacorl_amd/modules/tacorl/tacorl.py:

```python
import torch

from ... import encoder_stage as stage
from ... import image_ingest as ingest
from ... import ops
from ..._lib import call, ptr
from ...encoder_stage import image_flag
from ..common import register_views
from ..cql.cql_offline_lightning import CQL_Offline
from .latent_plan import LatentPlanShell


class TACORL(LatentPlanShell, CQL_Offline):
    def __init__(self, *args, **kwargs):
        self.action_loss_every_n_steps = kwargs.pop("action_loss_every_n_steps", 1)
        super().__init__(*args, **kwargs)

    def build_networks(self):
        from ..play_lmp.play_lmp_for_rl import PlayLMP, load_play_lmp

        lmp = self.__dict__.pop("_play_lmp", None)
        if lmp is None:
            lmp = load_play_lmp(self.play_lmp_dir, self.lmp_epoch_to_load, self.overwrite_lmp_cfg, device=self.dev,
                                compute_dtype=self.compute, image_dtype=self.img_dtype, unsafe_pickle=self.lmp_unsafe_pickle)
        assert isinstance(lmp, PlayLMP)
# ... 60 lines not shown
                                      and acts.shape == self.acts.shape))):
            call("tacorl_stage_transition", ptr(disp), dd, ptr(self.reward), ptr(e.done), B,
                 ptr(acts) if acts is not None else None, ptr(self.acts) if acts is not None else None,
                 acts.numel() if acts is not None else 0, ops.stream())
        else:
            if acts is not None:
                self.acts.copy_(acts)
            self.reward.copy_(disp == 1)
            e.done.copy_(self.reward)
        e.set_noise(noise)

    def _fold_ok(self, f, c, T, batch):
        e, hw = self.engine, f.hw[c]
        if not (f.form == "f32_nchw" and f.aug is None and T >= 2 and e.use_fused and stage.fused_fwd_ok(hw, self.compute, self.img_dtype)):
            return False
        goal = batch["goal"][c] if c in e.cams else None
        if c in e.cams and not (c in e.slot and list(e.slot[c]) == ["obs", "goal", "next"] and goal.is_cuda and goal.is_contiguous()
                                and goal.dtype == torch.float32 and ingest.vector_ok(
                [ingest.PackJob(goal.data_ptr(), 3 * hw[0] * hw[1], 0, 1)], f.form, hw)):
            return False
        v, simg = f.frames[c], 3 * hw[0] * hw[1]
        return stage.SourceTable.ok(v.data_ptr(), simg, hw) and stage.SourceTable.ok(v.data_ptr() + 4 * (T - 1) * simg, T * simg, hw)

    def _stage_frames(self, batch, noise, nchw=True, fold=False):
        from ...data.replay import wait_ready

        wait_ready(batch)
        f = ingest.window_form(batch, nchw)
        B, T, hw, aug = f.B, f.T, f.hw, f.aug
        self.engine.extra_normal = {"eps_pr": (B, self.action_dim)}
        self.engine.ensure_batch(B, {c: hw[c] for c in self.engine.cams})
        self.eps_pr = self.engine.extra_noise["eps_pr"]
        self._ensure_seq(B, T, hw)
        e = self.engine
        if self.ad is not None and (getattr(self, "acts", None) is None or self.acts.shape[:2] != (B, T)):
            ops.note_alloc()
            self.acts = torch.zeros(B, T, 7, device=self.dev)
        if getattr(self, "_stage_stream", None) is None:
            self._stage_stream = torch.cuda.Stream(device=self.dev)
        main = torch.cuda.current_stream()
        side = self._stage_stream if getattr(self, "stage_side", True) else main
        side.wait_stream(main)
        with torch.cuda.stream(side):
            self._stage_small(batch, noise, B, T)
        u8, Job, ip = f.form in ingest.U8_FORMS, ingest.PackJob, None if f.ids is None else f.ids.data_ptr()
        cams_all = sorted(set(self.all_modalities) | set(e.cams))
        for c in cams_all:
            v = f.frames[c]
            assert v.is_cuda and v.is_contiguous() and v.dtype == (torch.uint8 if u8 else torch.float32)
        folded = tuple(c for c in cams_all if fold and self._fold_ok(f, c, T, batch))
        if folded != self._folded:
            ops.note_alloc()
            self._folded = folded
        self.frames.drop()
        e.X3.drop()
        e.fp_src = {c: {"next": self.src_tbl[c].entry(1)} for c in folded if c in e.cams}
        for x in e.extra_enc:
            x["src"] = self.src_tbl[x["cam"]].entry(0) if x["cam"] in folded else None
        for c in cams_all:
            v = f.frames[c]
            src, simg = v.data_ptr(), 3 * f.src_hw[c][0] * f.src_hw[c][1]
            if c in folded:
                self.src_tbl[c].fill([(src, simg), (src + 4 * (T - 1) * simg, T * simg)], hw[c])
                form, shw = f.form, f.src_hw[c]
                later = lambda jobs, c=c, keep=v, form=form, shw=shw: ingest.pack(jobs, form, self.img_dtype, shw, hw[c])
                if c in self.all_modalities:
                    self.frames.defer(c, lambda c=c, later=later, src=src, simg=simg: later([Job(src, simg, self.frames.raw(c).data_ptr(), B * T)]))
                if c in e.cams:
                    x3, slot = e.X3.raw(c).data_ptr(), B * 3 * hw[c][0] * hw[c][1] * e.X3.raw(c).element_size()
                    ingest.pack([Job(src, T * simg, x3, B), Job(batch["goal"][c].data_ptr(), simg, x3 + slot, B)], form, self.img_dtype, shw, hw[c])
                    e.X3.defer(c, lambda later=later, src=src, simg=simg, x3=x3, slot=slot: later([Job(src + 4 * (T - 1) * simg, T * simg, x3 + 2 * slot, B)]))
                continue
            jobs, roles = [], []
            if c in self.all_modalities:
                jobs, roles = [Job(src, simg, self.frames.raw(c).data_ptr(), B * T, ip, 1)], ["window"]
            if c in e.cams:
                x3, slot = e.X3.raw(c).data_ptr(), B * 3 * hw[c][0] * hw[c][1] * e.X3.raw(c).element_size()
                if ip is not None:
                    jobs += [Job(src, simg, x3, B, ip, T), Job(src, simg, x3 + slot, B, ip + 8 * B * T, 1),
                             Job(src, simg, x3 + 2 * slot, B, ip + 8 * (T - 1), T)]
                else:
                    g = batch["goal"][c]
                    assert g.is_cuda and g.is_contiguous() and g.dtype == v.dtype
                    jobs += [Job(src, T * simg, x3, B), Job(g.data_ptr(), simg, x3 + slot, B),
                             Job(src + v.element_size() * (T - 1) * simg, T * simg, x3 + 2 * slot, B)]
                roles += ["obs", "goal", "next"]
            if aug is not None:
                jobs = [j._replace(**ingest.window_tables(aug, c, r, T)) for j, r in zip(jobs, roles)]
            if len(jobs) == 4 and T >= 2 and ingest.vector_ok(jobs, f.form, hw[c]):
                ingest.pack_window(jobs, T, self.img_dtype, hw[c])
            else:
                ingest.pack(jobs, f.form, self.img_dtype, f.src_hw[c], hw[c], aug["pad"][c] if aug is not None else None)
        main.wait_stream(side)
        return B, T, hw

    def _ad_due(self):
        k = self.action_loss_every_n_steps
        return self.ad is not None and (self.finetune_action_decoder or k <= 1 or (self._step_count + 1) % k == 0)

    def _device_front(self, B, T, hw, optimize, with_ad=True):
        e = self.engine
        ops.mark("front:start")
        if getattr(self, "_pr_stream", None) is None:
            self._pr_stream, self._side_stream = torch.cuda.Stream(device=self.dev), torch.cuda.Stream(device=self.dev)
        main = torch.cuda.current_stream()
        mods = self.plan_recognition_modalities
        emb, ld = (self.f_out[mods[0]], 32) if len(mods) == 1 else (self.pr_in, self.pr_in.shape[1])
        ad_prep, ad_prepared = None, False
        if (with_ad and optimize and self.finetune_action_decoder and getattr(self, "ad_early_prepare", True)
                and self.ad._bwd_fast(B, self.compute)):
            self._side_stream.wait_stream(main)
            with torch.cuda.stream(self._side_stream):
                self.ad.refresh_mirrors(B, T - 1)
                ad_prepared = self.ad.prepare_backward(B, T - 1, self.compute)
                ad_prep = torch.cuda.Event()
                ad_prep.record(self._side_stream)
        split = with_ad and (T >= 24 or (optimize and self.finetune_action_decoder))
        forked = []

        def fork_branches():
            forked.append(self._fork_pr_ad(B, T, main, mods, emb, ld, with_ad, optimize, ad_prep, ad_prepared))

        if not (split and e.encode_split(fork_branches)):
            e._encode_all()
        ops.mark("front:encoded")
        if not forked:
            fork_branches()
        ready, ad_on_side = forked[0]
        e.action_ready = ready
        e.phase_a(encoded=True, optimize=optimize)
        if ad_prep is not None:
            main.wait_stream(self._side_stream)
        segmented = self._segmented() or not self._use_graph
        if with_ad and not ad_on_side:
            if segmented:
                main.wait_stream(self._pr_stream)
            else:
                self._ad_join = self._pr_stream
        if segmented:
            main.wait_stream(self._pr_stream)
            e.action_ready = None
            self._join_ad()

    def _fork_pr_ad(self, B, T, main, mods, emb, ld, with_ad, optimize, ad_prep, ad_prepared):
        e = self.engine
        self._ad_join = None
        ad_on_side = with_ad and not (optimize and self.finetune_action_decoder)
        self._pr_stream.wait_stream(main)
        with torch.cuda.stream(self._pr_stream):
            ops.mark("pr:start")
            if len(mods) > 1:
                for j, c in enumerate(mods):
                    ops.copy_cols(self.f_out[c], 0, 32, self.pr_in, 32 * j, self.pr_in.shape[1], B * T, 32)
            self.pr.forward(emb, ld, B, T, self.compute, inference=True, sample=(self.eps_pr, self.plan), frozen=True)
            ops.mark("pr:plan")
            ready = torch.cuda.Event()
            ready.record(self._pr_stream)
            if with_ad and not ad_on_side:
                if ad_prep is not None:
                    self._pr_stream.wait_event(ad_prep)
                self.ad.loss_step(self, self.acts, self.plan, B, T, True, defer_update=self._defer_ad_update(),
                                  mirrors_current=ad_prep is not None, prepared=ad_prepared)
        if ad_on_side:
            self._side_stream.wait_event(ready)
            with torch.cuda.stream(self._side_stream):
                ops.mark("ad:start")
                self.ad.loss_step(self, self.acts, self.plan, B, T, False, frozen=not self.finetune_action_decoder)
                ops.mark("ad:end")
            self._ad_join = self._side_stream
        return ready, ad_on_side

    def get_pr_latent_plan(self, batch, noise=None, nchw=True):
        B, T, hw = self._stage_frames(batch, noise, nchw)
        xd = image_flag(self.img_dtype)
        for c in self.all_modalities:
            H, W = hw[c]
            call("tacorl_encoder_fwd", 1, ops.ptr_array([self.frames[c]]), ops.ptr_array([self.lmp_net.enc(c)]),
                 ops.ptr_array([self.f_out[c]]), ops.ptr_array([self.f_act[c]]), ops.int_array([B * T]), H, W, xd,
                 self.compute, ops.stream())
        for j, c in enumerate(self.plan_recognition_modalities):
            ops.copy_cols(self.f_out[c], 0, 32, self.pr_in, 32 * j, self.pr_in.shape[1], B * T, 32)
        head = self.pr.forward(self.pr_in, self.pr_in.shape[1], B, T, self.compute, inference=True)
        call("tacorl_pr_sample", ptr(head), ptr(self.eps_pr), ptr(self.plan), None, None, B, self.action_dim,
             float(self.pr.min_std), ops.stream())
        return self.plan

    def _step(self, batch, noise, optimize, log_type, nchw=True):
        B, T, hw = self._stage_frames(batch, noise, nchw, fold=getattr(self, "fp32_ingest", True))
        with_ad = self._ad_due()
        key = ("tacorl", B, T, tuple(sorted(hw.items())), self.current_epoch < self.bc_epochs, optimize, with_ad)
        e, bc = self.engine, self.current_epoch < self.bc_epochs
        ad_update = with_ad and optimize and self.finetune_action_decoder and self._defer_ad_update()

        def tail():
            e.phase_c(optimize)
            self._join_ad()
            if ad_update:
                self.ad.update(self)
            ops.mark("step:end")

        segmented = self._segmented()
        ad_ft = optimize and self.finetune_action_decoder
        ad_side = with_ad and segmented and self._use_graph
        side = None
        if ad_side and ad_ft:
            side = (0, lambda: self.ad.loss_step(self, self.acts, self.plan, B, T, True, defer_update=True), 1)
        elif ad_side:
            side = (0, lambda: self.ad.loss_step(self, self.acts, self.plan, B, T, False, frozen=not self.finetune_action_decoder))
        def allreduce_grads():
            if ad_update:
                self._join_ad()
            e.allreduce_grads()

        self._run_segments(key, [lambda: self._device_front(B, T, hw, optimize, with_ad and not ad_side),
                                 lambda: e.phase_b(bc, optimize), tail],
                           [e.allreduce_alpha, allreduce_grads], side=side)
        self._publish_logs(log_type, extra=("action_loss",) if with_ad else ())
```

tacorl_amd/networks/action_decoder.py:

```python
import ctypes as C

import torch

from .. import ops
from .._lib import ACT_NONE, ACT_RELU, call, ptr
from ..blocks import TensorBlock


RNN_MAXP = 4


class RowsState:

    @property
    def hidden(self):
        return self.h[self.flip]


class ActionDecoderLogistic:
    def __init__(self, device, state_dim=32, goal_dim=32, latent_plan_dim=16, hidden_size=256, out_features=7,
                 act_max_bound=(1.0,) * 7, act_min_bound=(-1.0,) * 7, gripper_alpha=1.0, policy_rnn_dropout_p=0.0,
                 num_layers=2, rnn_model="rnn_decoder", discrete_gripper=True, include_goal=False, num_classes=10,
                 n_mixtures=10, **unused):
        if rnn_model != "rnn_decoder" or include_goal or policy_rnn_dropout_p != 0.0:
# ... 139 lines not shown
        R, H, L, blk = state.R, self.hidden, self.L, self.blk
        if plan.shape != (R, self.P) or emb.shape != (R, self.E) or plan.dtype != torch.float32 or emb.dtype != torch.float32:
            raise ValueError(f"step_rows takes fp32 plan ({R}, {self.P}) and emb ({R}, {self.E}), got {tuple(plan.shape)} and "
                             f"{tuple(emb.shape)}")
        if not (plan.is_contiguous() and emb.stride(1) == 1 and plan.device == state.x.device == emb.device):
            raise ValueError("step_rows takes device tensors with contiguous rows")
        flags, any_restart = self._restart_flags(state, restart)
        call("tacorl_build_ad_input", ptr(plan), ptr(emb), emb.stride(0), ptr(state.x), R, 1, 1, self.P, self.E, ops.stream())
        prev, new = state.h[state.flip], state.h[state.flip ^ 1]
        if self.rows_route(R) == "composed":
            self._step_rows_composed(state, prev, new, flags if any_restart else None)
        else:
            x, K = state.x, self.P + self.E
            for l in range(L):
                call("tacorl_rows_linear2_fwd", ptr(x), K, K, blk.p(f"rnn.weight_ih_l{l}"), blk.p(f"rnn.bias_ih_l{l}"), ptr(prev[l]),
                     H, H, blk.p(f"rnn.weight_hh_l{l}"), blk.p(f"rnn.bias_hh_l{l}"), ptr(flags), ptr(new[l]), H, R, H,
                     ACT_RELU, ops.stream())
                x, K = new[l], H
            call("tacorl_rows_linear2_fwd", ptr(x), H, H, blk.p("mean_fc.weight"), blk.p("mean_fc.bias"), None, 0, 0, None, None,
                 None, ptr(state.heads), state.heads.shape[1], R, self.NH, ACT_NONE, ops.stream())
        if noise is not None:
            state.ra.copy_(noise[0].reshape(state.ra.shape))
            state.rb.copy_(noise[1].reshape(state.rb.shape))
        else:
            state.ra.uniform_()
            state.rb.uniform_()
        call("tacorl_logistic_mixture_sample" if self.discrete_gripper else "tacorl_logistic_mixture_nogrip_sample",
             ptr(state.heads), state.heads.shape[1], ptr(state.ra), ptr(state.rb), ptr(state.out), R, self.Da, self.K, ops.stream())
        state.flip ^= 1
        return state.out

    def _ensure(self, B, Tm):
        if self._shape == (B, Tm):
            return
        ops.note_alloc()
        f = lambda *s: torch.zeros(*s, device=self.dev)
        R, H = B * Tm, self.hidden
        self.x_seq = f(R, self.P + self.E)
        self.xin = [f(R, H) for _ in range(self.L)]
        self.h = [f(R, H) for _ in range(self.L)]
        self.h0 = f(B, H)
        self.NHP = (self.NH + 31) // 32 * 32
        self.heads, self.d_heads = f(R, self.NHP), f(R, self.NHP)
        self.ws = torch.empty(max(256, ops.L.lib().tacorl_logistic_mixture_ws_bytes(B, Tm, self.Da)), dtype=torch.uint8,
                              device=self.dev)
        nb = ops.L.lib().tacorl_linear_add_fwd_ws_bytes(1, ops.int_array([B]), H, H)
        self.rnn_ws = torch.empty(max(256, nb), dtype=torch.uint8, device=self.dev)
        bf = lambda *s: torch.zeros(*s, device=self.dev, dtype=torch.bfloat16)
        self.hb = [bf((R + 63) // 64 * 64, H) for _ in range(self.L)]
        self.h0b = bf(B, H)
        self.whb = [bf(H, H) for _ in range(self.L)]
        self.wib = [None] + [bf(H, H) for _ in range(1, self.L)]
        self.headw_b, self.headb = bf(self.NHP, H), f(self.NHP)
        self.xb_seq, self.wih0_b = bf(R, 128), bf(H, 128)
        self._mirror_shape = self._bf16_version = None
        self._shape = (B, Tm)

    def twin_ok(self, B, compute):
        H, K = self.hidden, self.P + self.E
        return (compute == ops.BF16 and bool(ops.L.lib().tacorl_rnn_linear_supported(B, H, H)) and 32 <= K <= 64
                and K % 8 == 0 and H % 16 == 0 and getattr(self, "fused_input_proj", True) and getattr(self, "twin_pass", True))

    def twin_state(self, B, Tm):
        tw = getattr(self, "_twin", None)
        if tw is None or tw.shape != (B, Tm):
            ops.note_alloc()
            self._ensure(B, Tm)
            R, H = B * Tm, self.hidden
            f = lambda *s: torch.zeros(*s, device=self.dev)
            bf = lambda *s: torch.zeros(*s, device=self.dev, dtype=torch.bfloat16)
            tw = self._twin = type("TwinPass", (), {})()
            tw.shape = (B, Tm)
            tw.xin, tw.h, tw.hb = [f(R, H) for _ in range(self.L)], [f(R, H) for _ in range(self.L)], [bf(R, H) for _ in range(self.L)]
            tw.heads = f(R, self.NHP)
            tw.xb_seq = bf(R, 128)
            tw.ws = torch.empty(self.ws.numel(), dtype=torch.uint8, device=self.dev)
        return tw

    def _ring_proj(self):
        return self.P + self.E <= 128

    def twin_input_proj(self, plan, emb, ld_emb, B, T, Tm):
        tw, blk = self.twin_state(B, Tm), self.blk
        if self._ring_proj():
            call("tacorl_build_ad_input_bf16", ptr(plan), ptr(emb), ld_emb, ptr(tw.xb_seq), B, T, Tm, self.P, self.E, ops.stream())
            return tw
        call("tacorl_ad_input_proj", ptr(plan), ptr(emb), ld_emb, blk.p("rnn.weight_ih_l0"), blk.p("rnn.bias_ih_l0"),
             ptr(tw.xin[0]), B, T, Tm, self.P, self.E, self.hidden, ops.stream())
        return tw

    def refresh_mirrors(self, B, Tm):
        self._ensure(B, Tm)
        blk, H = self.blk, self.hidden
        srcs = ([blk.p(f"rnn.weight_hh_l{l}") for l in range(self.L)] + [blk.p(f"rnn.weight_ih_l{l}") for l in range(1, self.L)]
                + [blk.p("mean_fc.weight")])
        dsts = self.whb + self.wib[1:] + [self.headw_b]
        call("tacorl_to_bf16_batch", len(srcs), ops.ptr_array(srcs), ops.ptr_array(dsts),
             (C.c_long * len(srcs))(*([H * H] * (len(srcs) - 1) + [self.NH * H])), ops.stream())
        self._mirror_ring, self._mirror_shape = self._ring_proj(), (B, Tm)
        if self._mirror_ring:
            call("tacorl_pad_to_bf16", blk.p("rnn.weight_ih_l0"), self.P + self.E, ptr(self.wih0_b), 128, H, self.P + self.E, ops.stream())
        ob = blk.off["mean_fc.bias"][0]
        self.headb[: self.NH].copy_(blk.param[ob: ob + self.NH])

    def prepare_backward(self, B, Tm, compute):
        if not self._bwd_fast(B, compute):
            return False
        self._ensure(B, Tm)
        self._ensure_bptt(B, Tm)
        self._transpose_weights()
        if self._heads_ring(B * Tm):
            call("tacorl_transpose_pad_to_bf16", self.blk.p("mean_fc.weight"), ptr(self.headwt_b), self.NH, self.hidden,
                 self.headwt_b.shape[1], ops.stream())
        return True

    def _bwd_fast(self, B, compute):
        H = self.hidden
        return compute == ops.BF16 and bool(ops.L.lib().tacorl_rnn_linear_supported(B, H, H)) and H % 32 == 0

    def _heads_ring(self, R):
        KP = (self.NH + 127) // 128 * 128
        ok = getattr(self, "heads_dgrad_ring", True) and bool(ops.L.lib().tacorl_rnn_linear_supported(R, KP, self.hidden))
        if ok and getattr(self, "_hd_shape", None) != (R, KP):
            ops.note_alloc()
            self.d_heads_b = torch.zeros((R + 63) // 64 * 64, KP, device=self.dev, dtype=torch.bfloat16)
            self.headwt_b = torch.zeros(self.hidden, KP, device=self.dev, dtype=torch.bfloat16)
            self._hd_shape = (R, KP)
        return ok

    def _ensure_bptt(self, B, Tm):
        if getattr(self, "_bptt_shape", None) != (B, Tm):
            ops.note_alloc()
            H, L, R = self.hidden, self.L, B * Tm
            bf = lambda *s: torch.zeros(*s, device=self.dev, dtype=torch.bfloat16)
            self.DZb = [bf(R, H) for _ in range(L)]
            self.whtb = [bf(H, H) for _ in range(L)]
            self.wihtb = [None] + [bf(H, H) for _ in range(1, L)]
            self._bptt_shape = (B, Tm)

    def twin_heads(self, twin, B, Tm):
        if getattr(twin, "heads_done", False):
            return
        call("tacorl_rnn_linear_fwd", ptr(twin.hb[self.L - 1]), ptr(self.headw_b), ptr(self.headb), None, 0, ptr(twin.heads), None,
             B * Tm, self.hidden, self.NHP, ACT_NONE, ops.stream())
        twin.heads_done = True

    def _lin(self, x, ldx, w, b, y, M, K, N, act, compute, ldy=None):
        nb = ops.L.lib().tacorl_linear_add_fwd_ws_bytes(1, ops.int_array([M]), K, N)
        ws = ops.workspace(nb, self.dev, "ad_splitk")
        call("tacorl_linear_add_fwd", 1, ops.ptr_array([x]), ldx, ops.ptr_array([w]), ops.ptr_array([b]), None, 0,
             ops.ptr_array([y]), N if ldy is None else ldy, ops.int_array([M]), K, N, act, compute, ptr(ws), ws.numel(),
             ops.stream())

    def forward(self, plan, emb, ld_emb, B, T, Tm, compute, frozen=False, mirrors_current=False, twin=None):
        self._ensure(B, Tm)
        blk, H, R = self.blk, self.hidden, B * Tm
        x, K = self.x_seq, self.P + self.E
        fast = compute == ops.BF16 and bool(ops.L.lib().tacorl_rnn_linear_supported(B, H, H))
        proj_fused = (fast and 32 <= K <= 64 and K % 8 == 0 and H % 16 == 0 and getattr(self, "fused_input_proj", True))
        ring = fast and self._ring_proj() and getattr(self, "fused_input_proj", True) and (proj_fused or twin is None)
        if not ((proj_fused or ring) and frozen):
            call("tacorl_build_ad_input", ptr(plan), ptr(emb), ld_emb, ptr(self.x_seq), B, T, Tm, self.P, self.E,
                 ops.stream())
        ver = blk.param._version
        fresh = ((frozen and getattr(self, "_bf16_version", None) == ver) or mirrors_current) and getattr(self, "_mirror_shape", None) == (B, Tm)
        if fast:
            self._bf16_version = ver if frozen else None
        if fast and getattr(self, "_mirror_ring", None) != self._ring_proj():
            fresh = False
        if fast and not fresh:
            self.refresh_mirrors(B, Tm)
        at = ops._at
        if fast:
            if ring:
                call("tacorl_build_ad_input_bf16", ptr(plan), ptr(emb), ld_emb, ptr(self.xb_seq), B, T, Tm, self.P, self.E, ops.stream())
            elif proj_fused:
                call("tacorl_ad_input_proj", ptr(plan), ptr(emb), ld_emb, blk.p("rnn.weight_ih_l0"), blk.p("rnn.bias_ih_l0"),
                     ptr(self.xin[0]), B, T, Tm, self.P, self.E, H, ops.stream())
            else:
                self._lin(x, K, blk.p("rnn.weight_ih_l0"), blk.p("rnn.bias_ih_l0"), self.xin[0], R, K, H, ACT_NONE, compute)
            L = self.L
            assert twin is None or (proj_fused and twin.shape == (B, Tm)), "twin pass: twin_ok() / twin_state(B, Tm)"
            hbp = lambda l, t, o=self: C.c_void_p(o.hb[l].data_ptr() + 2 * t * B * H)
            xbp = lambda t, o=self: C.c_void_p(o.xb_seq.data_ptr() + 2 * t * B * 128)
            for s_ in range(Tm + 2 * (L - 1)):
                xs, wt, bs, ad, ys, yb, ac = [], [], [], [], [], [], []
                x2, ad2, y2, yb2 = [], [], [], []
                xe, xe2, we, b2 = [], [], [], []
                for l in range(L):
                    t = s_ - 2 * l
                    if 0 <= t < Tm:
                        ext = ring and l == 0
                        xs.append(ptr(self.h0b) if t == 0 else hbp(l, t - 1)); wt.append(ptr(self.whb[l]))
                        bs.append(blk.p(f"rnn.bias_hh_l{l}")); ad.append(None if ext else at(self.xin[l], t * B * H))
                        ys.append(at(self.h[l], t * B * H)); yb.append(hbp(l, t)); ac.append(ACT_RELU)
                        xe.append(xbp(t) if ext else None); we.append(ptr(self.wih0_b) if ext else None)
                        b2.append(blk.p("rnn.bias_ih_l0") if ext else None)
                        if twin is not None:
                            x2.append(ptr(self.h0b) if t == 0 else hbp(l, t - 1, twin))
                            ad2.append(None if ext else at(twin.xin[l], t * B * H))
                            y2.append(at(twin.h[l], t * B * H)); yb2.append(hbp(l, t, twin))
                            xe2.append(xbp(t, twin) if ext else None)
                    t = s_ - 2 * l + 1
                    if l >= 1 and 0 <= t < Tm:
                        xs.append(hbp(l - 1, t)); wt.append(ptr(self.wib[l])); bs.append(blk.p(f"rnn.bias_ih_l{l}"))
                        ad.append(None); ys.append(at(self.xin[l], t * B * H)); yb.append(None); ac.append(ACT_NONE)
                        xe.append(None); we.append(None); b2.append(None)
                        if twin is not None:
                            x2.append(hbp(l - 1, t, twin)); ad2.append(None); y2.append(at(twin.xin[l], t * B * H)); yb2.append(None)
                            xe2.append(None)
                for i in range(0, len(xs), RNN_MAXP):
                    c = lambda a, i=i: ops.ptr_array(a[i: i + RNN_MAXP])
                    n, acs = len(xs[i: i + RNN_MAXP]), ops.int_array(ac[i: i + RNN_MAXP])
                    tw_ = twin is not None
                    if ring:
                        call("tacorl_rnn_linear_fwd_batch_ext", n, c(xs), c(x2) if tw_ else None, c(wt), c(bs), c(ad),
                             c(ad2) if tw_ else None, H, c(ys), c(y2) if tw_ else None, c(yb), c(yb2) if tw_ else None,
                             B, B if tw_ else 0, H, H, acs, c(xe), c(xe2) if tw_ else None, c(we), c(b2), ops.stream())
                    elif tw_:
                        call("tacorl_rnn_linear_fwd_batch_twin", n, c(xs), c(x2), c(wt), c(bs), c(ad), c(ad2), H, c(ys), c(y2),
                             c(yb), c(yb2), B, B, H, H, acs, ops.stream())
                    else:
                        call("tacorl_rnn_linear_fwd_batch", n, c(xs), c(wt), c(bs), c(ad), H, c(ys), c(yb), B, H, H, acs,
                             ops.stream())
            x, K = self.h[L - 1], H
        for l in range(self.L if fast else 0, self.L):
            self._lin(x, K, blk.p(f"rnn.weight_ih_l{l}"), blk.p(f"rnn.bias_ih_l{l}"), self.xin[l], R, K, H, ACT_NONE,
                      compute)
            for t in range(Tm):
                prev = self.h0 if t == 0 else at(self.h[l], (t - 1) * B * H)
                call("tacorl_linear_add_fwd", 1, ops.ptr_array([prev]), H, ops.ptr_array([blk.p(f"rnn.weight_hh_l{l}")]),
                     ops.ptr_array([blk.p(f"rnn.bias_hh_l{l}")]), ops.ptr_array([at(self.xin[l], t * B * H)]), H,
                     ops.ptr_array([at(self.h[l], t * B * H)]), H, ops.int_array([B]), H, H, ACT_RELU, compute,
                     ptr(self.rnn_ws), self.rnn_ws.numel(), ops.stream())
            x, K = self.h[l], H
        if fast:
            if twin is not None and not getattr(self, "twin_heads_apart", True):
                call("tacorl_rnn_linear_fwd_batch_twin", 1, ops.ptr_array([self.hb[self.L - 1]]), ops.ptr_array([twin.hb[self.L - 1]]),
                     ops.ptr_array([self.headw_b]), ops.ptr_array([self.headb]), None, None, 0, ops.ptr_array([self.heads]),
                     ops.ptr_array([twin.heads]), None, None, R, R, H, self.NHP, ops.int_array([ACT_NONE]), ops.stream())
                twin.heads_done = True
                return
            if twin is not None:
                twin.heads_done = False
            call("tacorl_rnn_linear_fwd", ptr(self.hb[self.L - 1]), ptr(self.headw_b), ptr(self.headb), None, 0,
                 ptr(self.heads), None, R, H, self.NHP, ACT_NONE, ops.stream())
        else:
            self._lin(x, H, blk.p("mean_fc.weight"), blk.p("mean_fc.bias"), self.heads, R, H, self.NH, ACT_NONE, compute,
                      ldy=self.NHP)

    def loss(self, actions, loss_out, B, T, Tm, want_grad, grad_scale=1.0, twin=None, lazy=False):
        heads, ws = (self.heads, self.ws) if twin is None else (twin.heads, twin.ws)
        d_heads = ptr(self.d_heads) if want_grad and twin is None else None
        if self.discrete_gripper:
            call("tacorl_logistic_mixture_loss", ptr(heads), self.NHP, ptr(actions), d_heads, None if lazy else loss_out, B, T, Tm,
                 self.Da, self.K, self.num_classes, float(self.gripper_alpha), float(grad_scale), ptr(ws), ws.numel(), ops.stream())
        else:
            call("tacorl_logistic_mixture_nogrip_loss", ptr(heads), self.NHP, ptr(actions), d_heads, None if lazy else loss_out, B, T,
                 Tm, self.Da, self.K, self.num_classes, float(grad_scale), ptr(ws), ws.numel(), ops.stream())
        self._lazy_loss = (ws, B, Tm, loss_out) if lazy else None

    def finish_loss(self):
        pend = getattr(self, "_lazy_loss", None)
        if pend is not None:
            ws, B, Tm, loss_out = pend
            call("tacorl_logistic_mixture_finish" if self.discrete_gripper else "tacorl_logistic_mixture_nogrip_finish", ptr(ws),
                 ws.numel(), B, Tm, self.Da, loss_out, ops.stream())

    def loss_step(self, module, actions, plan, B, T, optimize, frozen=False, defer_update=False, mirrors_current=False,
                  prepared=False, emb=None):
        from .._lib import LOG_SLOTS

        acts = actions
        cams = module.action_decoder_modalities if emb is None else None
        if emb is not None:
            emb, ld = emb
        elif len(cams) == 1:
            emb, ld = module.f_out[cams[0]], 32
        elif cams == module.plan_recognition_modalities:
            emb, ld = module.pr_in, module.pr_in.shape[1]
        else:
            if getattr(module, "_ad_in", None) is None or module._ad_in.shape[0] != B * T:
                ops.note_alloc()
                module._ad_in = torch.zeros(B * T, 32 * len(cams), device=self.dev)
            for j, c in enumerate(cams):
                ops.copy_cols(module.f_out[c], 0, 32, module._ad_in, 32 * j, module._ad_in.shape[1], B * T, 32)
            emb, ld = module._ad_in, module._ad_in.shape[1]
        self.forward(plan, emb, ld, B, T, T - 1, module.compute, frozen=frozen and not optimize, mirrors_current=mirrors_current)
        slot = ops._at(module.engine.logs, LOG_SLOTS.index("action_loss"))
        self.loss(acts, slot, B, T, T - 1, want_grad=optimize, grad_scale=1.0 / module.world_size, lazy=True)
        if optimize:
            self.backward(B, T - 1, module.compute, need_input_grad=False, wavefront=getattr(self, "finetune_wavefront", True),
                          prepared=prepared)
            if not defer_update:
                self.update(module)

    def update(self, module):
        ops.adam_step(self.blk.param, self.blk.grad, self.blk.m, self.blk.v, module.action_decoder_lr, 0.0, self.blk.step)

    def _wgrad(self, x, ldx, dz, ld_dz, M, K, O, dw, db, compute):
        nb = ops.L.lib().tacorl_linear_wgrad_ws_bytes(1, ops.int_array([M]), K, O)
        ws = ops.workspace(nb, self.dev, "ad_wgrad")
        call("tacorl_linear_wgrad", 1, ops.ptr_array([x]), ldx, ops.ptr_array([dz]), ld_dz, ops.int_array([M]), K, O,
             ops.ptr_array([dw]), ops.ptr_array([db]) if db is not None else None, 0, compute, ptr(ws), ws.numel(),
             ops.stream())

    def _dgrad(self, dz, ld_dz, w, out, ld_out, M, O, I, compute, src=None, ld_src=0, act=ACT_NONE, addend=None,
               ld_add=0):
        nb = ops.L.lib().tacorl_linear_dgrad_ws_bytes(1, ops.int_array([M]), O, I)
        ws = ops.workspace(nb, self.dev, "ad_dgrad")
        call("tacorl_linear_dgrad_splitk", 1, ops.ptr_array([dz]), ld_dz, ops.ptr_array([w]), ops.ptr_array([out]), ld_out,
             ops.ptr_array([src]) if src is not None else None, ld_src, act,
             ops.ptr_array([addend]) if addend is not None else None, ld_add, ops.int_array([M]), O, I, compute,
             ptr(ws), ws.numel(), ops.stream())

    def _square_wgrads(self, B, Tm):
        blk, H, R, L = self.blk, self.hidden, B * Tm, self.L
        sup = ops.L.lib().tacorl_rnn_wgrad_supported
        if (not getattr(self, "wgrad_batched", True) or Tm < 2 or 2 * L - 1 > 4 or L < 2
                or not sup((Tm - 1) * B, H, H) or not sup(R, H, H)):
            return False
        bfp = lambda t, off: C.c_void_p(t.data_ptr() + 2 * off)
        dz, x, rows, dw, db = [], [], [], [], []
        for l in range(L):
            dz.append(bfp(self.DZb[l], B * H)); x.append(ptr(self.hb[l])); rows.append((Tm - 1) * B)
            dw.append(blk.g(f"rnn.weight_hh_l{l}")); db.append(None)
        for l in range(1, L):
            dz.append(ptr(self.DZb[l])); x.append(ptr(self.hb[l - 1])); rows.append(R)
            dw.append(blk.g(f"rnn.weight_ih_l{l}")); db.append(blk.g(f"rnn.bias_ih_l{l}"))
        call("tacorl_rnn_wgrad_batch", len(dz), ops.ptr_array(dz), H, ops.ptr_array(x), H, ops.int_array(rows), H, H,
             ops.ptr_array(dw), ops.ptr_array(db), 0, ops.stream())
        return True

    def _layer_wgrads(self, l, B, Tm, compute, fast, square_done=False):
        blk, H, R = self.blk, self.hidden, B * Tm
        if square_done:
            if l == 0:
                self._wgrad(self.x_seq, self.P + self.E, self.DZ[0], H, R, self.P + self.E, H, blk.g("rnn.weight_ih_l0"),
                            blk.g("rnn.bias_ih_l0"), compute)
            call("tacorl_copy_cols", blk.g(f"rnn.bias_ih_l{l}"), H, blk.g(f"rnn.bias_hh_l{l}"), H, 1, H, 0, 0, ops.stream())
            return
        h, DZ, at = self.h[l], self.DZ[l], ops._at
        tr = lambda rows: fast and bool(ops.L.lib().tacorl_rnn_wgrad_supported(rows, H, H))
        bfp = lambda t, off: C.c_void_p(t.data_ptr() + 2 * off)
        if Tm > 1 and tr((Tm - 1) * B):
            call("tacorl_rnn_wgrad", bfp(self.DZb[l], B * H), H, ptr(self.hb[l]), H, (Tm - 1) * B, H, H,
                 blk.g(f"rnn.weight_hh_l{l}"), None, 0, ops.stream())
        elif Tm > 1:
            self._wgrad(h, H, at(DZ, B * H), H, (Tm - 1) * B, H, H, blk.g(f"rnn.weight_hh_l{l}"), None, compute)
        else:
            blk.grad_views[f"rnn.weight_hh_l{l}"].zero_()
        xin, K = (self.x_seq, self.P + self.E) if l == 0 else (self.h[l - 1], H)
        if l > 0 and Tm > 1 and tr(R):
            call("tacorl_rnn_wgrad", ptr(self.DZb[l]), H, ptr(self.hb[l - 1]), H, R, H, H, blk.g(f"rnn.weight_ih_l{l}"),
                 blk.g(f"rnn.bias_ih_l{l}"), 0, ops.stream())
        else:
            self._wgrad(xin, K, DZ, H, R, K, H, blk.g(f"rnn.weight_ih_l{l}"), blk.g(f"rnn.bias_ih_l{l}"), compute)
        call("tacorl_copy_cols", blk.g(f"rnn.bias_ih_l{l}"), H, blk.g(f"rnn.bias_hh_l{l}"), H, 1, H, 0, 0,
             ops.stream())

    def _bptt_wavefront(self, B, Tm, prepared=False):
        blk, H, L = self.blk, self.hidden, self.L
        at = ops._at
        bfp = lambda t, off: C.c_void_p(t.data_ptr() + 2 * off)
        row = lambda t: t * B * H
        if not prepared:
            self._transpose_weights()
        top, last = L - 1, row(Tm - 1)
        call("tacorl_relu_mask_mul", at(self.dHs[top], last), None, at(self.h[top], last), at(self.DZ[top], last), B * H, ops.stream())
        call("tacorl_to_bf16_batch", 1, ops.ptr_array([at(self.DZ[top], last)]), ops.ptr_array([bfp(self.DZb[top], last)]),
             (C.c_long * 1)(B * H), ops.stream())
        for s_ in range(Tm - 1 + 2 * (L - 1)):
            xs, wt, ad, ms, ys, yb = [], [], [], [], [], []
            for l in range(L):
                j = s_ - 2 * (L - 1 - l)
                if j < 0:
                    continue
                u = Tm - 2 - j
                if u >= 0:
                    xs.append(bfp(self.DZb[l], row(u + 1))); wt.append(ptr(self.whtb[l])); ad.append(at(self.dHs[l], row(u)))
                    ms.append(at(self.h[l], row(u))); ys.append(at(self.DZ[l], row(u))); yb.append(bfp(self.DZb[l], row(u)))
                t = Tm - 1 - j
                if l >= 1 and t >= 0:
                    xs.append(bfp(self.DZb[l], row(t))); wt.append(ptr(self.wihtb[l])); ad.append(None)
                    if t == Tm - 1:
                        ms.append(at(self.h[l - 1], row(t))); ys.append(at(self.DZ[l - 1], row(t))); yb.append(bfp(self.DZb[l - 1], row(t)))
                    else:
                        ms.append(None); ys.append(at(self.dHs[l - 1], row(t))); yb.append(None)
            if xs:
                call("tacorl_rnn_linear_bwd_batch", len(xs), ops.ptr_array(xs), ops.ptr_array(wt), ops.ptr_array(ad), H,
                     ops.ptr_array(ms), ops.ptr_array(ys), ops.ptr_array(yb), B, H, H, ops.stream())

    def _transpose_weights(self):
        blk, H = self.blk, self.hidden
        srcs = [blk.p(f"rnn.weight_hh_l{l}") for l in range(self.L)] + [blk.p(f"rnn.weight_ih_l{l}") for l in range(1, self.L)]
        dsts = [self.whtb[l] for l in range(self.L)] + [self.wihtb[l] for l in range(1, self.L)]
        for i in range(0, len(srcs), 16):
            n = len(srcs[i: i + 16])
            call("tacorl_transpose_to_bf16_batch", n, ops.ptr_array(srcs[i: i + 16]), ops.ptr_array(dsts[i: i + 16]),
                 ops.int_array([H] * n), ops.int_array([H] * n), ops.stream())

    def backward(self, B, Tm, compute, need_input_grad=False, wgrad_stream=None, join=True, wavefront=True, prepared=False):
        blk, H, R, L = self.blk, self.hidden, B * Tm, self.L
        if getattr(self, "_bshape", None) != (B, Tm):
            ops.note_alloc()
            f = lambda *s: torch.zeros(*s, device=self.dev)
            self.dHs = [f(R, H) for _ in range(L)]
            self.dH = self.dHs[L - 1]
            self.DZ = [f(R, H) for _ in range(L)]
            self.dx_seq = f(R, self.P + self.E)
            self._bshape = (B, Tm)
        at = ops._at

        def side(fn):
            if wgrad_stream is None:
                return fn()
            wgrad_stream.wait_stream(torch.cuda.current_stream())
            with torch.cuda.stream(wgrad_stream):
                fn()

        fast = self._bwd_fast(B, compute)
        ring = fast and self._heads_ring(R)
        if ring:
            KP = self.headwt_b.shape[1]
            if not prepared:
                call("tacorl_transpose_pad_to_bf16", blk.p("mean_fc.weight"), ptr(self.headwt_b), self.NH, H, KP, ops.stream())
            call("tacorl_pad_to_bf16", ptr(self.d_heads), self.NHP, ptr(self.d_heads_b), KP, R, self.NH, ops.stream())
        Rp = (R + 63) // 64 * 64
        slabs = max(d for d in range(1, 9) if (Rp // 64) % d == 0)
        if (ring and getattr(self, "heads_wgrad_slabs", True) and H % 128 == 0
                and bool(ops.L.lib().tacorl_rnn_wgrad_supported(Rp // slabs, self.headwt_b.shape[1], H))):
            def heads_wgrad():
                KP = self.headwt_b.shape[1]
                nb = ops.L.lib().tacorl_rnn_wgrad_slabs_ws_bytes(slabs, KP, H)
                ws = ops.workspace(nb, self.dev, "ad_heads_wgrad")
                call("tacorl_rnn_wgrad_slabs", ptr(self.d_heads_b), KP, ptr(self.hb[L - 1]), H, Rp, KP, H, self.NH, slabs,
                     blk.g("mean_fc.weight"), blk.g("mean_fc.bias"), 0, ptr(ws), ws.numel(), ops.stream())
            side(heads_wgrad)
        else:
            side(lambda: self._wgrad(self.h[L - 1], H, self.d_heads, self.NHP, R, H, self.NH, blk.g("mean_fc.weight"),
                                     blk.g("mean_fc.bias"), compute))
# ... 46 lines not shown
```

tacorl_amd/networks/plan_recognition.py:

```python
import torch

from .. import ops
from .._lib import ACT_NONE, ACT_RELU, call, ptr
from ..blocks import TensorBlock


class PlanRecognition:
    def __init__(self, state_dim, latent_plan_dim, device, num_heads=8, num_layers=2, encoder_hidden_size=2048,
                 fc_hidden_size=4096, max_position_embeddings=16, min_std=1e-4, dropout_p=0.0, trainable=True,
                 **unused):
        self.D_in = state_dim
        self.pad = (-state_dim) % num_heads
        self.D = state_dim + self.pad
        self.A, self.H, self.L = latent_plan_dim, num_heads, num_layers
        self.FF, self.FC, self.T_max, self.min_std = encoder_hidden_size, fc_hidden_size, max_position_embeddings, min_std
        self.latent_plan_dim = latent_plan_dim
        self.dropout_p = dropout_p
        D, FF, FC, A = self.D, self.FF, self.FC, self.A
        spec = [("position_embeddings.weight", (self.T_max, D)), ("layernorm.weight", (D,)), ("layernorm.bias", (D,))]
        for l in range(num_layers):
            p = f"transformer_encoder.layers.{l}."
            spec += [(p + "self_attn.in_proj_weight", (3 * D, D)), (p + "self_attn.in_proj_bias", (3 * D,)),
                     (p + "self_attn.out_proj.weight", (D, D)), (p + "self_attn.out_proj.bias", (D,)),
                     (p + "linear1.weight", (FF, D)), (p + "linear1.bias", (FF,)),
                     (p + "linear2.weight", (D, FF)), (p + "linear2.bias", (D,)),
                     (p + "norm1.weight", (D,)), (p + "norm1.bias", (D,)),
                     (p + "norm2.weight", (D,)), (p + "norm2.bias", (D,))]
        spec += [("fc.weight", (FC, D)), ("fc.bias", (FC,)), ("mean_fc.weight", (A, FC)),
                 ("variance_fc.weight", (A, FC)), ("mean_fc.bias", (A,)), ("variance_fc.bias", (A,))]
        self.blk = TensorBlock(spec, device, trainable=trainable)
        self.dev = device
        self._shape = None

    def _ensure(self, B, T):
        if self._shape == (B, T):
            return
        if T > self.T_max:
            raise ValueError(f"sequence length {T} > max_position_embeddings {self.T_max}")
        ops.note_alloc()
        f = lambda *s: torch.zeros(*s, device=self.dev)
        R, D = B * T, self.D
        self.x = [f(R, D) for _ in range(2 * self.L + 1)]
        self.qkv = [f(R, 3 * D) for _ in range(self.L)]
        self.att = [f(R, D) for _ in range(self.L)]
        self.proj = [f(R, D) for _ in range(self.L)]
        self.ff1 = [f(R, self.FF) for _ in range(self.L)]
        self.ff2 = [f(R, D) for _ in range(self.L)]
        self.stats = [f(R, 2) for _ in range(2 * self.L)]
        self.pooled, self.fc_out, self.head = f(B, D), f(B, self.FC), f(B, 2 * self.A)
        self.keep = self.keep_flat = self.keep_entries = None
        if self.dropout_p > 0:
            from ..noise import dropout_id
            per = [T * D]
            for _ in range(self.L):
                per += [self.H * T * T, T * D, T * self.FF, T * D]
            offs, o = [], 0
            for n_ in per:
                offs.append(o)
                o += (B * n_ + 3) // 4 * 4
            self.keep_flat = torch.ones(o, dtype=torch.uint8, device=self.dev)
            self.keep = [self.keep_flat[o_: o_ + B * n_] for o_, n_ in zip(offs, per)]
            self.keep_entries = [(dropout_id(i), o_, n_, 1.0 - self.dropout_p) for i, (o_, n_) in enumerate(zip(offs, per))]
        self._shape = (B, T)

    def stage_dropout(self, B, T, masks=None):
        self._ensure(B, T)
        if self.keep is None:
            return
        if masks is None:
            for k in self.keep:
                k.bernoulli_(1.0 - self.dropout_p)
            return
        assert len(masks) == len(self.keep), (len(masks), len(self.keep))
        for i, (k, m) in enumerate(zip(self.keep, masks)):
            m = m.to(self.dev)
            if (i - 1) % 4 != 0 or i == 0:
                m = m.permute(1, 0, 2)
            k.copy_(m.reshape(-1).to(torch.uint8))

    def _drop(self, x, i, n):
        call("tacorl_dropout_mul", ptr(x), ptr(self.keep[i]), 1.0 / (1.0 - self.dropout_p), n, ops.stream())

    def _lin(self, x, ldx, w, b, y, M, K, N, act, compute):
        nb = ops.L.lib().tacorl_linear_add_fwd_ws_bytes(1, ops.int_array([M]), K, N)
        ws = ops.workspace(nb, self.dev, "lin_splitk")
        call("tacorl_linear_add_fwd", 1, ops.ptr_array([x]), ldx, ops.ptr_array([w]), ops.ptr_array([b]), None, 0,
             ops.ptr_array([y]), N, ops.int_array([M]), K, N, act, compute, ptr(ws), ws.numel(), ops.stream())

    def _fused_offsets(self):
        names = ["position_embeddings.weight"]
        for l in range(self.L):
            p = f"transformer_encoder.layers.{l}."
            names += [p + k for k in ("self_attn.in_proj_weight", "self_attn.in_proj_bias", "self_attn.out_proj.weight",
                                      "self_attn.out_proj.bias", "linear1.weight", "linear1.bias", "linear2.weight",
                                      "linear2.bias", "norm1.weight", "norm1.bias", "norm2.weight", "norm2.bias")]
        return [self.blk.off[n][0] for n in names]

    def fused_inference_ok(self, T, ld_emb, compute):
        return bool(compute == ops.BF16 and self.pad == 0 and ld_emb % 4 == 0 and 2 * self.A <= 64
                    and ops.L.lib().tacorl_pr_encoder_fused_supported(self.D, T, self.H, self.FF, self.L))

    def prepare_inference(self):
        import ctypes as C
        blk = self.blk
        if getattr(self, "_pb", None) is None:
            ops.note_alloc()
            self._pb = torch.zeros(blk.param.numel(), device=self.dev, dtype=torch.bfloat16)
            self._foff = (C.c_long * (1 + 12 * self.L))(*self._fused_offsets())
            self._Wc = torch.zeros(2 * self.A, self.D, device=self.dev)
            self._bc = torch.zeros(2 * self.A, device=self.dev)
        n4 = blk.param.numel() // 4 * 4
        call("tacorl_to_bf16_batch", 1, ops.ptr_array([blk.param]), ops.ptr_array([self._pb]), (C.c_long * 1)(n4),
             ops.stream())
        call("tacorl_pr_head_compose", blk.p("fc.weight"), blk.p("fc.bias"), blk.p("mean_fc.weight"), blk.p("mean_fc.bias"),
             ptr(self._Wc), ptr(self._bc), self.D, self.FC, 2 * self.A, ops.stream())

    def forward(self, emb, ld_emb, B, T, compute, inference=False, sample=None, prepared=False, frozen=False, train=False):
        self._ensure(B, T)
        blk, D, R = self.blk, self.D, B * T
        drop = self._dropping = bool(train and not inference and self.dropout_p > 0)
        ks = 1.0 / (1.0 - self.dropout_p) if drop else 1.0
        if inference and self.fused_inference_ok(T, ld_emb, compute):
            ver = blk.param._version
            if not prepared and not (frozen and getattr(self, "_prep_version", None) == ver):
                self.prepare_inference()
                self._prep_version = ver if frozen else None
            if sample is not None:
                eps, plan = sample
                call("tacorl_pr_encoder_fused_sample", ptr(emb), ld_emb, ptr(blk.param), ptr(self._pb), self._foff,
                     ptr(self.pooled), B, D, T, self.H, self.FF, self.L, ptr(self._Wc), ptr(self._bc), ptr(eps),
                     ptr(self.head), ptr(plan), self.A, float(self.min_std), ops.stream())
                return self.head
            call("tacorl_pr_encoder_fused", ptr(emb), ld_emb, ptr(blk.param), ptr(self._pb), self._foff, ptr(self.pooled),
                 B, D, T, self.H, self.FF, self.L, ops.stream())
            self._lin(self.pooled, D, blk.p("fc.weight"), blk.p("fc.bias"), self.fc_out, B, D, self.FC, ACT_NONE, compute)
            self._lin(self.fc_out, self.FC, blk.p("mean_fc.weight"), blk.p("mean_fc.bias"), self.head, B, self.FC,
                      2 * self.A, ACT_NONE, compute)
            return self.head
        if (not inference and not drop and getattr(self, "fused_train", True) and self.fused_inference_ok(T, ld_emb, compute)
                and ops.L.lib().tacorl_pr_encoder_fused_train_supported(self.D, T, self.H, self.FF, self.L)):
            import ctypes as C
            if not prepared:
                if getattr(self, "_pb", None) is None:
                    ops.note_alloc()
                    self._pb = torch.zeros(blk.param.numel(), device=self.dev, dtype=torch.bfloat16)
                    self._foff = (C.c_long * (1 + 12 * self.L))(*self._fused_offsets())
                    self._Wc = torch.zeros(2 * self.A, self.D, device=self.dev)
                    self._bc = torch.zeros(2 * self.A, device=self.dev)
                call("tacorl_to_bf16_batch", 1, ops.ptr_array([blk.param]), ops.ptr_array([self._pb]),
                     (C.c_long * 1)(blk.param.numel() // 4 * 4), ops.stream())
            self._prep_version = None
            save = []
            for l in range(self.L):
                save += [self.x[2 * l], self.qkv[l], self.att[l], self.proj[l], self.x[2 * l + 1], self.ff1[l], self.ff2[l],
                         self.stats[2 * l], self.stats[2 * l + 1]]
            self._fused_saved = (B, T)
            self._composed = bool(prepared and sample is not None and 2 * self.A <= 64 and getattr(self, "composed_head", True))
            if self._composed:
                eps, plan = sample
                call("tacorl_pr_encoder_fused_train_sample", ptr(emb), ld_emb, ptr(blk.param), ptr(self._pb), self._foff,
                     ptr(self.pooled), B, D, T, self.H, self.FF, self.L, ops.ptr_array(save), ptr(self._Wc), ptr(self._bc),
                     ptr(eps), ptr(self.head), ptr(plan), self.A, float(self.min_std), ops.stream())
                return self.head
            call("tacorl_pr_encoder_fused_train", ptr(emb), ld_emb, ptr(blk.param), ptr(self._pb), self._foff, ptr(self.pooled),
                 B, D, T, self.H, self.FF, self.L, ops.ptr_array(save), ops.stream())
            self._lin(self.pooled, D, blk.p("fc.weight"), blk.p("fc.bias"), self.fc_out, B, D, self.FC, ACT_NONE, compute)
            self._lin(self.fc_out, self.FC, blk.p("mean_fc.weight"), blk.p("mean_fc.bias"), self.head, B, self.FC,
                      2 * self.A, ACT_NONE, compute)
            if sample is not None:
                eps, plan = sample
                call("tacorl_pr_sample", ptr(self.head), ptr(eps), ptr(plan), None, None, B, self.A, float(self.min_std),
                     ops.stream())
            return self.head
        self._fused_saved, self._composed = None, False
        call("tacorl_add_rows_bcast", ptr(emb), ld_emb, blk.p("position_embeddings.weight"), ptr(self.x[0]), R, T,
             self.D_in, D, ops.stream())
        if drop:
            self._drop(self.x[0], 0, R * D)
        for l in range(self.L):
            p = f"transformer_encoder.layers.{l}."
            xin, x1, x2 = self.x[2 * l], self.x[2 * l + 1], self.x[2 * l + 2]
            self._lin(xin, D, blk.p(p + "self_attn.in_proj_weight"), blk.p(p + "self_attn.in_proj_bias"), self.qkv[l],
                      R, D, 3 * D, ACT_NONE, compute)
            if drop:
                call("tacorl_attention_dropout_fwd", ptr(self.qkv[l]), ptr(self.att[l]), ptr(self.keep[1 + 4 * l]), ks, B, T,
                     D, self.H, ops.stream())
            else:
                call("tacorl_attention_fwd", ptr(self.qkv[l]), ptr(self.att[l]), B, T, D, self.H, ops.stream())
            self._lin(self.att[l], D, blk.p(p + "self_attn.out_proj.weight"), blk.p(p + "self_attn.out_proj.bias"),
                      self.proj[l], R, D, D, ACT_NONE, compute)
            if drop:
                self._drop(self.proj[l], 2 + 4 * l, R * D)
            call("tacorl_add_layernorm_fwd", ptr(xin), ptr(self.proj[l]), blk.p(p + "norm1.weight"),
                 blk.p(p + "norm1.bias"), ptr(x1), ptr(self.stats[2 * l]), R, D, 1e-5, ops.stream())
            self._lin(x1, D, blk.p(p + "linear1.weight"), blk.p(p + "linear1.bias"), self.ff1[l], R, D, self.FF,
                      ACT_RELU, compute)
            if drop:
                self._drop(self.ff1[l], 3 + 4 * l, R * self.FF)
            self._lin(self.ff1[l], self.FF, blk.p(p + "linear2.weight"), blk.p(p + "linear2.bias"), self.ff2[l], R,
                      self.FF, D, ACT_NONE, compute)
            if drop:
                self._drop(self.ff2[l], 4 + 4 * l, R * D)
            call("tacorl_add_layernorm_fwd", ptr(x1), ptr(self.ff2[l]), blk.p(p + "norm2.weight"),
                 blk.p(p + "norm2.bias"), ptr(x2), ptr(self.stats[2 * l + 1]), R, D, 1e-5, ops.stream())
        call("tacorl_mean_over_t", ptr(self.x[2 * self.L]), ptr(self.pooled), B, T, D, ops.stream())
        self._lin(self.pooled, D, blk.p("fc.weight"), blk.p("fc.bias"), self.fc_out, B, D, self.FC, ACT_NONE, compute)
        self._lin(self.fc_out, self.FC, blk.p("mean_fc.weight"), blk.p("mean_fc.bias"), self.head, B, self.FC,
                  2 * self.A, ACT_NONE, compute)
        if sample is not None:
            eps, plan = sample
            call("tacorl_pr_sample", ptr(self.head), ptr(eps), ptr(plan), None, None, B, self.A, float(self.min_std),
                 ops.stream())
        return self.head

    def _wgrad(self, x, ldx, dz, ld_dz, M, K, O, dw, db, compute):
        nb = ops.L.lib().tacorl_linear_wgrad_ws_bytes(1, ops.int_array([M]), K, O)
        ws = ops.workspace(nb, self.dev, "lin_wgrad")
        call("tacorl_linear_wgrad", 1, ops.ptr_array([x]), ldx, ops.ptr_array([dz]), ld_dz, ops.int_array([M]), K, O,
             ops.ptr_array([dw]), ops.ptr_array([db]), 0, compute, ptr(ws), ws.numel(), ops.stream())

    def _wgrad_n(self, xs, ldx, dzs, ld_dz, M, K, O, dws, dbs, compute):
        n = len(xs)
        nb = ops.L.lib().tacorl_linear_wgrad_ws_bytes(n, ops.int_array([M] * n), K, O)
        ws = ops.workspace(nb, self.dev, "lin_wgrad")
        call("tacorl_linear_wgrad", n, ops.ptr_array(xs), ldx, ops.ptr_array(dzs), ld_dz, ops.int_array([M] * n), K, O,
             ops.ptr_array(dws), ops.ptr_array(dbs), 0, compute, ptr(ws), ws.numel(), ops.stream())

    def _dgrad(self, dz, ld_dz, w, out, ld_out, M, O, I, compute, src=None, ld_src=0, act=ACT_NONE, addend=None,
               ld_add=0):
        nb = ops.L.lib().tacorl_linear_dgrad_ws_bytes(1, ops.int_array([M]), O, I)
        ws = ops.workspace(nb, self.dev, "lin_dgrad")
        call("tacorl_linear_dgrad_splitk", 1, ops.ptr_array([dz]), ld_dz, ops.ptr_array([w]), ops.ptr_array([out]), ld_out,
             ops.ptr_array([src]) if src is not None else None, ld_src, act,
             ops.ptr_array([addend]) if addend is not None else None, ld_add, ops.int_array([M]), O, I, compute,
             ptr(ws), ws.numel(), ops.stream())

    def _ln_bwd(self, dy, x, res, w, stats, dv, dw, db, R, D):
        nb = ops.L.lib().tacorl_add_layernorm_bwd_ws_bytes(R, D)
        ws = ops.workspace(nb, self.dev, "ln_bwd")
        call("tacorl_add_layernorm_bwd", ptr(dy), ptr(x), ptr(res), w, ptr(stats), ptr(dv), dw, db, R, D, 0, ptr(ws),
             ws.numel(), ops.stream())

    def prepare_backward(self, B):
        blk, D, FF = self.blk, self.D, self.FF
        if getattr(self, "_wt", None) is None or self._lnpart.numel() != self.L * 2 * B * 64:
            ops.note_alloc()
            bf = lambda n: torch.zeros(n, device=self.dev, dtype=torch.bfloat16)
            self._wt = [t for _ in range(self.L) for t in (bf(FF * D), bf(FF * D), bf(D * D), bf(3 * D * D))]
            self._lnpart = torch.zeros(self.L * 2 * B * 64, device=self.dev)
        srcs, shp = [], []
        for l in range(self.L):
            p = f"transformer_encoder.layers.{l}."
            srcs += [blk.p(p + "linear1.weight"), blk.p(p + "linear2.weight"), blk.p(p + "self_attn.out_proj.weight"), blk.p(p + "self_attn.in_proj_weight")]
            shp += [(FF, D), (D, FF), (D, D), (3 * D, D)]
        for i in range(0, len(srcs), 16):
            j = slice(i, i + 16)
            call("tacorl_transpose_to_bf16_batch", len(srcs[j]), ops.ptr_array(srcs[j]), ops.ptr_array(self._wt[j]),
                 ops.int_array([r for r, _ in shp[j]]), ops.int_array([c for _, c in shp[j]]), ops.stream())

    def backward(self, d_head, B, T, compute, wgrad_stream=None, prepared=False):
        blk, D, R, FF, FC, A2 = self.blk, self.D, B * T, self.FF, self.FC, 2 * self.A
        if getattr(self, "_bshape", None) != (B, T):
            ops.note_alloc()
            f = lambda *s: torch.zeros(*s, device=self.dev)
            per = lambda *s: [f(*s) for _ in range(self.L)]
            self.d_fc, self.d_pool = f(B, FC), f(B, D)
            self.dx, self.d_x1, self.d_att = f(R, D), f(R, D), f(R, D)
            self.dv, self.dv1, self.d_ff1, self.d_qkv = per(R, D), per(R, D), per(R, FF), per(R, 3 * D)
            self.dvb, self.dv1b = per(R, D), per(R, D)
            self._bshape = (B, T)

        def side(fn):
            if wgrad_stream is None:
                return fn()
            wgrad_stream.wait_stream(torch.cuda.current_stream())
            with torch.cuda.stream(wgrad_stream):
                fn()

        fused = (getattr(self, "_fused_saved", None) == (B, T) and getattr(self, "fused_backward", True)
                 and not getattr(self, "_dropping", False) and T == 16)
        wt_ready = None
# ... 110 lines not shown
```

Baseline: 1291 grad-steps/s.

## Fuse action-decoder bf16 input-row build into plan-recognition sampling kernel

The fused plan-recognition sampling kernel now also writes the action decoder's bf16 ring input rows: idle waves copy the embedding columns and wave 0 broadcasts the sampled plan. The separate build_ad_input_bf16 launch is then skipped on the frozen path. Inside the encoder, QKV projection and attention are split across all four waves rather than each wave computing every head redundantly, using a dedicated LDS buffer and dropping one barrier. The dead W2TOP prefetch branch is removed. The costs are more LDS, a full __syncthreads, and tighter coupling between the PR and AD modules.

```diff
diff --git a/include/tacorl_hip.h b/include/tacorl_hip.h
--- a/include/tacorl_hip.h
+++ b/include/tacorl_hip.h
@@ -281,6 +281,11 @@
                                    const long* offsets, float* pooled, int B, int D, int T, int H, int FF, int L,
                                    const float* Wc, const float* bc, const float* eps, float* head, float* plan,
                                    int A, float min_std, tacorl_stream_t stream);
+int tacorl_pr_encoder_fused_sample_rows(const float* emb, int ld_emb, const float* params, const void* params_bf16,
+                                        const long* offsets, float* pooled, int B, int D, int T, int H, int FF, int L,
+                                        const float* Wc, const float* bc, const float* eps, float* head, float* plan,
+                                        int A, float min_std, void* xb_seq, int Tm, int P, int E, const float* emb_ad,
+                                        int ld_ad, tacorl_stream_t stream);
 int tacorl_pr_encoder_fused_train(const float* emb, int ld_emb, const float* params, const void* params_bf16,
                                   const long* offsets, float* pooled, int B, int D, int T, int H, int FF, int L,
                                   float* const* save, tacorl_stream_t stream);
diff --git a/tacorl_amd/_lib.py b/tacorl_amd/_lib.py
--- a/tacorl_amd/_lib.py
+++ b/tacorl_amd/_lib.py
@@ -50,6 +50,8 @@
     "tacorl_pr_encoder_bwd_fused": (_i, [_p, _p, _p, _p, _p, _i, _p, _p, _p, _p, _p, _p, _i, _i, _i, _i, _i, _i, _p]),
     "tacorl_pr_encoder_fused_train_sample": (_i, [_p, _i, _p, _p, _p, _p, _i, _i, _i, _i, _i, _i, _p, _p, _p, _p, _p, _p, _i, _f, _p]),
     "tacorl_pr_encoder_fused_sample": (_i, [_p, _i, _p, _p, _p, _p, _i, _i, _i, _i, _i, _i, _p, _p, _p, _p, _p, _i, _f, _p]),
+    "tacorl_pr_encoder_fused_sample_rows": (_i, [_p, _i, _p, _p, _p, _p, _i, _i, _i, _i, _i, _i, _p, _p, _p, _p, _p, _i, _f,
+                                                _p, _i, _i, _i, _p, _i, _p]),
     "tacorl_pr_head_compose": (_i, [_p, _p, _p, _p, _p, _p, _i, _i, _i, _p]),
     "tacorl_to_bf16_batch": (_i, [_i, _p, _p, _p, _p]),
     "tacorl_mlp_bwd_fused_supported": (_i, [_i, _i, _p, _i, _i]),
diff --git a/tacorl_amd/csrc/pr_fused.hip b/tacorl_amd/csrc/pr_fused.hip
--- a/tacorl_amd/csrc/pr_fused.hip
+++ b/tacorl_amd/csrc/pr_fused.hip
@@ -6,9 +6,6 @@
 
 namespace {
 
-#ifndef PR_W2TOP
-#define PR_W2TOP 0
-#endif
 constexpr int PR_D = 32, PR_T = 16, PR_H = 8, PR_HD = 4, PR_MAXL = 4, PR_CH = 256;
 constexpr int XB_P = 40;
 constexpr int HB_P = 264;
@@ -33,6 +30,9 @@
   float min_std;
   PrSaveL sv[PR_MAXL];
   int save;
+  __bf16* xrow;
+  const float* xemb;
+  int x_ld, x_Tm, x_P, x_E;
 };
 
 __device__ __forceinline__ bf16x8 cvt8(const float* p) {
@@ -114,6 +114,7 @@
   __shared__ __attribute__((aligned(16))) __bf16 xb_s[4][T * XB_P];
   __shared__ __attribute__((aligned(16))) unsigned char big_s[4][T * HB_P * 2];
   const int lane = threadIdx.x & 63, w = threadIdx.x >> 6, i = lane & 15, g = lane >> 4;
+  __shared__ __attribute__((aligned(16))) __bf16 xatt[T * XB_P];
   __shared__ __attribute__((aligned(16))) float ypart[2][4][T * PR_D];
   constexpr int PR_B1C = 2;
   __shared__ __attribute__((aligned(16))) float b1_s[4][PR_B1C * PR_CH];
@@ -152,18 +153,21 @@
   };
   const int nchunk = a.FF / PR_CH;
   const bool sv0 = a.save && w == 0;
+  const int qt = w >> 1;
+  const bool svq = a.save && (g >> 1) == (w & 1);
   long rrow[RT];
 #pragma unroll
   for (int rt = 0; rt < RT; rt++) rrow[rt] = (long)b * T + 16 * rt + i;
   for (int l = 0; l < a.L; l++) {
     const PrLayerOff& o = a.l[l];
     const PrSaveL& S = a.sv[l];
-    bf16x8 inw[6], outw[2];
-    f32x4 inb[6], outb[2], n1w[2], n1b[2], n2w[2], n2b[2], b2v[2];
-#pragma unroll
-    for (int nt = 0; nt < 6; nt++) {
-      inw[nt] = *reinterpret_cast<const bf16x8*>(a.Pb + o.in_w + (long)(16 * nt + i) * PR_D + 8 * g);
-      inb[nt] = *reinterpret_cast<const f32x4*>(a.P + o.in_b + 16 * nt + 4 * g);
+    bf16x8 inw[3], outw[2];
+    f32x4 inb[3], outb[2], n1w[2], n1b[2], n2w[2], n2b[2], b2v[2];
+#pragma unroll
+    for (int k3 = 0; k3 < 3; k3++) {
+      const int nt = 2 * k3 + qt;
+      inw[k3] = *reinterpret_cast<const bf16x8*>(a.Pb + o.in_w + (long)(16 * nt + i) * PR_D + 8 * g);
+      inb[k3] = *reinterpret_cast<const f32x4*>(a.P + o.in_b + 16 * nt + 4 * g);
     }
 #pragma unroll
     for (int nt = 0; nt < 2; nt++) {
@@ -190,13 +194,6 @@
         b1pre[j] = *reinterpret_cast<const f32x4*>(a.P + o.b1 + PR_CH * (c < nchunk ? c : c0) + 4 * lane);
       }
     }
-    if (RT == 1 && PR_W2TOP) {
-#pragma unroll
-      for (int ks = 0; ks < 8; ks++)
-#pragma unroll
-        for (int nt = 0; nt < 2; nt++)
-          w2f[ks][nt] = *reinterpret_cast<const bf16x8*>(W2 + (long)(16 * nt + i) * a.FF + PR_CH * c0 + 32 * ks + 8 * g);
-    }
     if (sv0) {
 #pragma unroll
       for (int rt = 0; rt < RT; rt++)
@@ -211,23 +208,23 @@
 #pragma unroll
       for (int rt = 0; rt < RT; rt++) xf[rt] = *reinterpret_cast<const bf16x8*>(xb + (16 * rt + i) * XB_P + 8 * g);
 #pragma unroll
-      for (int nt = 0; nt < 6; nt++) {
-        const bf16x8 wf = inw[nt];
-        const f32x4 bias = inb[nt];
+      for (int k3 = 0; k3 < 3; k3++) {
+        const int nt = 2 * k3 + qt;
+        const bf16x8 wf = inw[k3];
+        const f32x4 bias = inb[k3];
 #pragma unroll
         for (int rt = 0; rt < RT; rt++) {
           f32x4 acc = bias;
           acc = __builtin_amdgcn_mfma_f32_16x16x32_bf16(wf, xf[rt], acc, 0, 0, 0);
           *reinterpret_cast<f32x4*>(qkv + (16 * rt + i) * QKV_P + 16 * nt + 4 * g) = acc;
-          if (sv0) *reinterpret_cast<f32x4*>(S.qkv + rrow[rt] * 3 * PR_D + 16 * nt + 4 * g) = acc;
+          if (svq) *reinterpret_cast<f32x4*>(S.qkv + rrow[rt] * 3 * PR_D + 16 * nt + 4 * g) = acc;
         }
       }
     }
     lds_sync();
     PR_STAMP(1);
-#pragma unroll
-    for (int j = 0; j < 2 * RT; j++) {
-      const int p = lane + 64 * j, h = p / T, qi = p % T;
+    {
+      const int p = lane & (2 * T - 1), h = 2 * w + p / T, qi = p % T;
       f32x4 q = *reinterpret_cast<const f32x4*>(qkv + qi * QKV_P + PR_HD * h);
 #pragma unroll
       for (int e = 0; e < 4; e++) q[e] *= 0.5f * 1.44269504088896341f;
@@ -250,15 +247,17 @@
 #pragma unroll
         for (int e = 0; e < 4; e++) ov[e] += pr * vv[e];
       }
-      *reinterpret_cast<bf16x4*>(xb + qi * XB_P + PR_HD * h) = bf16x4{(__bf16)ov[0], (__bf16)ov[1], (__bf16)ov[2], (__bf16)ov[3]};
-      if (sv0) *reinterpret_cast<f32x4*>(S.att + ((long)b * T + qi) * PR_D + PR_HD * h) = ov;
-    }
-    lds_sync();
+      if (lane < 2 * T) {
+        *reinterpret_cast<bf16x4*>(xatt + qi * XB_P + PR_HD * h) = bf16x4{(__bf16)ov[0], (__bf16)ov[1], (__bf16)ov[2], (__bf16)ov[3]};
+        if (a.save) *reinterpret_cast<f32x4*>(S.att + ((long)b * T + qi) * PR_D + PR_HD * h) = ov;
+      }
+    }
+    __syncthreads();
     PR_STAMP(2);
     {
       bf16x8 af[RT];
 #pragma unroll
-      for (int rt = 0; rt < RT; rt++) af[rt] = *reinterpret_cast<const bf16x8*>(xb + (16 * rt + i) * XB_P + 8 * g);
+      for (int rt = 0; rt < RT; rt++) af[rt] = *reinterpret_cast<const bf16x8*>(xatt + (16 * rt + i) * XB_P + 8 * g);
 #pragma unroll
       for (int nt = 0; nt < 2; nt++) {
         const bf16x8 wf = outw[nt];
@@ -280,7 +279,6 @@
         }
       }
     }
-    lds_sync();
     put_xb(x);
     lds_sync();
     PR_STAMP(3);
@@ -298,14 +296,12 @@
 #pragma unroll
       for (int nt = 0; nt < 2; nt++)
         y[rt][nt] = w == 0 ? b2v[nt] : f32x4{0.f, 0.f, 0.f, 0.f};
-    for (int c = w; c < nchunk; c += 4) {
-      if (RT != 1 || !PR_W2TOP || c != w) {
-#pragma unroll
-        for (int ks = 0; ks < 8; ks++)
-#pragma unroll
-          for (int nt = 0; nt < 2; nt++)
-            w2f[ks][nt] = *reinterpret_cast<const bf16x8*>(W2 + (long)(16 * nt + i) * a.FF + PR_CH * c + 32 * ks + 8 * g);
-      }
+    auto ffn_chunk = [&](const int c, const bool more) {
+#pragma unroll
+      for (int ks = 0; ks < 8; ks++)
+#pragma unroll
+        for (int nt = 0; nt < 2; nt++)
+          w2f[ks][nt] = *reinterpret_cast<const bf16x8*>(W2 + (long)(16 * nt + i) * a.FF + PR_CH * c + 32 * ks + 8 * g);
 #pragma unroll
       for (int nt = 0; nt < 16; nt++) {
         const f32x4 bias = b1_staged ? *reinterpret_cast<const f32x4*>(b1_s[w] + PR_CH * ((c - w) >> 2) + 16 * nt + 4 * g)
@@ -320,7 +316,7 @@
         }
       }
       lds_sync();
-      if (c + 4 < nchunk) {
+      if (more) {
 #pragma unroll
         for (int nt = 0; nt < 16; nt++)
           w1f[nt] = *reinterpret_cast<const bf16x8*>(W1 + (long)(PR_CH * (c + 4) + 16 * nt + i) * PR_D + 8 * g);
@@ -335,7 +331,8 @@
         }
       }
       lds_sync();
-    }
+    };
+    for (int c = w; c < nchunk; c += 4) ffn_chunk(c, c + 4 < nchunk);
     PR_STAMP(4);
     {
       float* yp = ypart[l & 1][w];
@@ -359,7 +356,20 @@
     for (int rt = 0; rt < RT; rt++) layer_norm32_r(x[rt], n2w, n2b, g, sv0 ? S.st2 + 2 * rrow[rt] : nullptr);
     PR_STAMP(5);
   }
-  if (w != 0) return;
+  if (w != 0) {
+    if (a.xrow) {
+      const int u0 = a.x_P >> 3, nu = 16 - u0, K = a.x_P + a.x_E;
+      for (int e = (int)threadIdx.x - 64; e < a.x_Tm * nu; e += 192) {
+        const int t = e / nu, c = 8 * (u0 + e - t * nu);
+        const float* er = a.xemb + ((long)b * T + t) * a.x_ld;
+        bf16x8 v;
+#pragma unroll
+        for (int j = 0; j < 8; j++) v[j] = (__bf16)(c + j < K ? er[c + j - a.x_P] : 0.f);
+        *reinterpret_cast<bf16x8*>(a.xrow + ((long)t * a.B + b) * 128 + c) = v;
+      }
+    }
+    return;
+  }
 #pragma unroll
   for (int nt = 0; nt < 2; nt++) {
     f32x4 s = x[0][nt];
@@ -387,9 +397,19 @@
   }
   if (lane < 2 * A) a.head[(long)b * 2 * A + lane] = h;
   const float vr = __shfl(h, (lane + A) & 63, 64);
+  float pl = 0.f;
   if (lane < A) {
     const float sd = (vr > 20.f ? vr : log1pf(expf(vr))) + a.min_std;
-    a.plan[(long)b * A + lane] = tanhf(h + heps * sd);
+    pl = tanhf(h + heps * sd);
+    a.plan[(long)b * A + lane] = pl;
+  }
+  if (!a.xrow) return;
+  if (lane < A) xb[lane] = (__bf16)pl;
+  lds_sync();
+  const int u0 = a.x_P >> 3;
+  for (int e = lane; e < a.x_Tm * u0; e += 64) {
+    const int t = e / u0, c = 8 * (e - t * u0);
+    *reinterpret_cast<bf16x8*>(a.xrow + ((long)t * a.B + b) * 128 + c) = *reinterpret_cast<const bf16x8*>(xb + c);
   }
 }
 
@@ -1010,10 +1030,12 @@
 extern "C" int tacorl_pr_encoder_fused_train_supported(int D, int T, int H, int FF, int L) {
   return D == PR_D && tacorl_pr_encoder_fused_supported(D, T, H, FF, L) ? 1 : 0;
 }
+struct PrRows { void* out; const float* emb; int ld, Tm, P, E; };
 static int pr_encoder_fused_launch(const float* emb, int ld_emb, const float* params, const void* params_bf16,
                                    const long* offsets, float* pooled, int B, int D, int T, int H, int FF, int L,
                                    const float* Wc, const float* bc, const float* eps, float* head, float* plan, int A,
-                                   float min_std, tacorl_stream_t stream, float* const* save = nullptr) {
+                                   float min_std, tacorl_stream_t stream, float* const* save = nullptr,
+                                   const PrRows* rows = nullptr) {
   if (!tacorl_pr_encoder_fused_supported(D, T, H, FF, L) || ld_emb % 4 || B < 1) return TACORL_EINVAL;
   if (((uintptr_t)emb | (uintptr_t)params | (uintptr_t)params_bf16 | (uintptr_t)pooled) & 15) return TACORL_EINVAL;
   PrArgs a{};
@@ -1030,6 +1052,12 @@
     if (!bc || !eps || !head || !plan || A < 1 || 2 * A > 64 || ((uintptr_t)Wc & 15)) return TACORL_EINVAL;
     a.Wc = Wc; a.bc = bc; a.eps = eps; a.head = head; a.plan = plan; a.A = A; a.min_std = min_std;
   }
+  if (rows) {
+    if (!Wc || D != PR_D || !rows->out || ((uintptr_t)rows->out & 15) || !rows->emb || rows->Tm < 1 || rows->Tm > T ||
+        rows->P != A || rows->P % 8 || rows->E < 1 || rows->P + rows->E > 128 || rows->ld < rows->E)
+      return TACORL_EINVAL;
+    a.xrow = (__bf16*)rows->out; a.xemb = rows->emb; a.x_ld = rows->ld; a.x_Tm = rows->Tm; a.x_P = rows->P; a.x_E = rows->E;
+  }
   if (save) {
     for (int l = 0; l < L; l++) {
       float* const* q = save + 9 * l;
@@ -1076,6 +1104,16 @@
   if (!Wc) return TACORL_EINVAL;
   return pr_encoder_fused_launch(emb, ld_emb, params, params_bf16, offsets, pooled, B, D, T, H, FF, L, Wc, bc, eps, head,
                                  plan, A, min_std, stream);
+}
+extern "C" int tacorl_pr_encoder_fused_sample_rows(const float* emb, int ld_emb, const float* params, const void* params_bf16,
+                                                   const long* offsets, float* pooled, int B, int D, int T, int H, int FF,
+                                                   int L, const float* Wc, const float* bc, const float* eps, float* head,
+                                                   float* plan, int A, float min_std, void* xb_seq, int Tm, int P, int E,
+                                                   const float* emb_ad, int ld_ad, tacorl_stream_t stream) {
+  if (!Wc) return TACORL_EINVAL;
+  const PrRows rows{xb_seq, emb_ad, ld_ad, Tm, P, E};
+  return pr_encoder_fused_launch(emb, ld_emb, params, params_bf16, offsets, pooled, B, D, T, H, FF, L, Wc, bc, eps, head,
+                                 plan, A, min_std, stream, nullptr, &rows);
 }
 extern "C" int tacorl_pr_head_compose(const float* w_fc, const float* b_fc, const float* w_head, const float* b_head,
                                       float* Wc, float* bc, int D, int FC, int A2, tacorl_stream_t stream) {
diff --git a/tacorl_amd/modules/tacorl/tacorl.py b/tacorl_amd/modules/tacorl/tacorl.py
--- a/tacorl_amd/modules/tacorl/tacorl.py
+++ b/tacorl_amd/modules/tacorl/tacorl.py
@@ -236,7 +236,15 @@
             if len(mods) > 1:
                 for j, c in enumerate(mods):
                     ops.copy_cols(self.f_out[c], 0, 32, self.pr_in, 32 * j, self.pr_in.shape[1], B * T, 32)
-            self.pr.forward(emb, ld, B, T, self.compute, inference=True, sample=(self.eps_pr, self.plan), frozen=True)
+            ad_rows = None
+            if (ad_on_side and not self.finetune_action_decoder and getattr(self, "pr_writes_ad_rows", True)
+                    and getattr(self.pr, "writes_ad_rows", False)):
+                xb_seq, ad_emb = self.ad.ring_rows(B, T - 1, self.compute), self.ad.module_emb(self, B, T, gather=False)
+                if xb_seq is not None and ad_emb is not None:
+                    ad_rows = (xb_seq, T - 1, self.ad.P, self.ad.E, ad_emb[0], ad_emb[1])
+            self.pr.forward(emb, ld, B, T, self.compute, inference=True, sample=(self.eps_pr, self.plan), frozen=True,
+                            **({} if ad_rows is None else {"ad_rows": ad_rows}))
+            rows_current = bool(getattr(self.pr, "rows_written", False))
             ops.mark("pr:plan")
             ready = torch.cuda.Event()
             ready.record(self._pr_stream)
@@ -249,7 +257,8 @@
             self._side_stream.wait_event(ready)
             with torch.cuda.stream(self._side_stream):
                 ops.mark("ad:start")
-                self.ad.loss_step(self, self.acts, self.plan, B, T, False, frozen=not self.finetune_action_decoder)
+                self.ad.loss_step(self, self.acts, self.plan, B, T, False, frozen=not self.finetune_action_decoder,
+                                  rows_current=rows_current)
                 ops.mark("ad:end")
             self._ad_join = self._side_stream
         return ready, ad_on_side
diff --git a/tacorl_amd/networks/action_decoder.py b/tacorl_amd/networks/action_decoder.py
--- a/tacorl_amd/networks/action_decoder.py
+++ b/tacorl_amd/networks/action_decoder.py
@@ -315,13 +315,40 @@
              ops.ptr_array([y]), N if ldy is None else ldy, ops.int_array([M]), K, N, act, compute, ptr(ws), ws.numel(),
              ops.stream())
 
-    def forward(self, plan, emb, ld_emb, B, T, Tm, compute, frozen=False, mirrors_current=False, twin=None):
+    def _route(self, B, compute, twin=None):
+        H, K = self.hidden, self.P + self.E
+        fast = compute == ops.BF16 and bool(ops.L.lib().tacorl_rnn_linear_supported(B, H, H))
+        proj_fused = (fast and 32 <= K <= 64 and K % 8 == 0 and H % 16 == 0 and getattr(self, "fused_input_proj", True))
+        ring = fast and self._ring_proj() and getattr(self, "fused_input_proj", True) and (proj_fused or twin is None)
+        return fast, proj_fused, ring
+
+    def ring_rows(self, B, Tm, compute):
+        if not self._route(B, compute)[2]:
+            return None
+        self._ensure(B, Tm)
+        return self.xb_seq
+
+    def module_emb(self, module, B, T, gather=True):
+        cams = module.action_decoder_modalities
+        if len(cams) == 1:
+            return module.f_out[cams[0]], 32
+        if cams == module.plan_recognition_modalities:
+            return module.pr_in, module.pr_in.shape[1]
+        if not gather:
+            return None
+        if getattr(module, "_ad_in", None) is None or module._ad_in.shape[0] != B * T:
+            ops.note_alloc()
+            module._ad_in = torch.zeros(B * T, 32 * len(cams), device=self.dev)
+        for j, c in enumerate(cams):
+            ops.copy_cols(module.f_out[c], 0, 32, module._ad_in, 32 * j, module._ad_in.shape[1], B * T, 32)
+        return module._ad_in, module._ad_in.shape[1]
+
+    def forward(self, plan, emb, ld_emb, B, T, Tm, compute, frozen=False, mirrors_current=False, twin=None, rows_current=False):
         self._ensure(B, Tm)
         blk, H, R = self.blk, self.hidden, B * Tm
         x, K = self.x_seq, self.P + self.E
-        fast = compute == ops.BF16 and bool(ops.L.lib().tacorl_rnn_linear_supported(B, H, H))
-        proj_fused = (fast and 32 <= K <= 64 and K % 8 == 0 and H % 16 == 0 and getattr(self, "fused_input_proj", True))
-        ring = fast and self._ring_proj() and getattr(self, "fused_input_proj", True) and (proj_fused or twin is None)
+        fast, proj_fused, ring = self._route(B, compute, twin)
+        assert not rows_current or (ring and frozen), "rows_current: the frozen ring route only (ring_rows)"
         if not ((proj_fused or ring) and frozen):
             call("tacorl_build_ad_input", ptr(plan), ptr(emb), ld_emb, ptr(self.x_seq), B, T, Tm, self.P, self.E,
                  ops.stream())
@@ -336,7 +363,8 @@
         at = ops._at
         if fast:
             if ring:
-                call("tacorl_build_ad_input_bf16", ptr(plan), ptr(emb), ld_emb, ptr(self.xb_seq), B, T, Tm, self.P, self.E, ops.stream())
+                if not rows_current:
+                    call("tacorl_build_ad_input_bf16", ptr(plan), ptr(emb), ld_emb, ptr(self.xb_seq), B, T, Tm, self.P, self.E, ops.stream())
             elif proj_fused:
                 call("tacorl_ad_input_proj", ptr(plan), ptr(emb), ld_emb, blk.p("rnn.weight_ih_l0"), blk.p("rnn.bias_ih_l0"),
                      ptr(self.xin[0]), B, T, Tm, self.P, self.E, H, ops.stream())
@@ -431,25 +459,13 @@
                  ws.numel(), B, Tm, self.Da, loss_out, ops.stream())
 
     def loss_step(self, module, actions, plan, B, T, optimize, frozen=False, defer_update=False, mirrors_current=False,
-                  prepared=False, emb=None):
+                  prepared=False, emb=None, rows_current=False):
         from .._lib import LOG_SLOTS
 
         acts = actions
-        cams = module.action_decoder_modalities if emb is None else None
-        if emb is not None:
-            emb, ld = emb
-        elif len(cams) == 1:
-            emb, ld = module.f_out[cams[0]], 32
-        elif cams == module.plan_recognition_modalities:
-            emb, ld = module.pr_in, module.pr_in.shape[1]
-        else:
-            if getattr(module, "_ad_in", None) is None or module._ad_in.shape[0] != B * T:
-                ops.note_alloc()
-                module._ad_in = torch.zeros(B * T, 32 * len(cams), device=self.dev)
-            for j, c in enumerate(cams):
-                ops.copy_cols(module.f_out[c], 0, 32, module._ad_in, 32 * j, module._ad_in.shape[1], B * T, 32)
-            emb, ld = module._ad_in, module._ad_in.shape[1]
-        self.forward(plan, emb, ld, B, T, T - 1, module.compute, frozen=frozen and not optimize, mirrors_current=mirrors_current)
+        emb, ld = emb if emb is not None else self.module_emb(module, B, T)
+        self.forward(plan, emb, ld, B, T, T - 1, module.compute, frozen=frozen and not optimize, mirrors_current=mirrors_current,
+                     rows_current=rows_current)
         slot = ops._at(module.engine.logs, LOG_SLOTS.index("action_loss"))
         self.loss(acts, slot, B, T, T - 1, want_grad=optimize, grad_scale=1.0 / module.world_size, lazy=True)
         if optimize:
diff --git a/tacorl_amd/networks/plan_recognition.py b/tacorl_amd/networks/plan_recognition.py
--- a/tacorl_amd/networks/plan_recognition.py
+++ b/tacorl_amd/networks/plan_recognition.py
@@ -6,6 +6,8 @@
 
 
 class PlanRecognition:
+    writes_ad_rows = True
+
     def __init__(self, state_dim, latent_plan_dim, device, num_heads=8, num_layers=2, encoder_hidden_size=2048,
                  fc_hidden_size=4096, max_position_embeddings=16, min_std=1e-4, dropout_p=0.0, trainable=True,
                  **unused):
@@ -115,7 +117,9 @@
         call("tacorl_pr_head_compose", blk.p("fc.weight"), blk.p("fc.bias"), blk.p("mean_fc.weight"), blk.p("mean_fc.bias"),
              ptr(self._Wc), ptr(self._bc), self.D, self.FC, 2 * self.A, ops.stream())
 
-    def forward(self, emb, ld_emb, B, T, compute, inference=False, sample=None, prepared=False, frozen=False, train=False):
+    def forward(self, emb, ld_emb, B, T, compute, inference=False, sample=None, prepared=False, frozen=False, train=False,
+                ad_rows=None):
+        self.rows_written = False
         self._ensure(B, T)
         blk, D, R = self.blk, self.D, B * T
         drop = self._dropping = bool(train and not inference and self.dropout_p > 0)
@@ -127,6 +131,15 @@
                 self._prep_version = ver if frozen else None
             if sample is not None:
                 eps, plan = sample
+                if ad_rows is not None and D == 32 and ad_rows[2] == self.A and self.A % 8 == 0 and ad_rows[1] <= T \
+                        and ad_rows[2] + ad_rows[3] <= 128 and ad_rows[5] >= ad_rows[3]:
+                    xb_seq, Tm, P, E, emb_ad, ld_ad = ad_rows
+                    call("tacorl_pr_encoder_fused_sample_rows", ptr(emb), ld_emb, ptr(blk.param), ptr(self._pb), self._foff,
+                         ptr(self.pooled), B, D, T, self.H, self.FF, self.L, ptr(self._Wc), ptr(self._bc), ptr(eps),
+                         ptr(self.head), ptr(plan), self.A, float(self.min_std), ptr(xb_seq), Tm, P, E, ptr(emb_ad), ld_ad,
+                         ops.stream())
+                    self.rows_written = True
+                    return self.head
                 call("tacorl_pr_encoder_fused_sample", ptr(emb), ld_emb, ptr(blk.param), ptr(self._pb), self._foff,
                      ptr(self.pooled), B, D, T, self.H, self.FF, self.L, ptr(self._Wc), ptr(self._bc), ptr(eps),
                      ptr(self.head), ptr(plan), self.A, float(self.min_std), ops.stream())
```

Result: faster. 1314 grad-steps/s, median of 6 (+1.8%).
